# picoexperiment/AutoBub3hs

Hardware: AMD Instinct MI355X
Metric: frames/s end-to-end detect @1280x1024 8-bit (higher is better)
Workload: dtype u8

## Files before the change

autobub3hs_amd/_lib.py:

```python
import ctypes as C
import os
import subprocess

HERE = os.path.dirname(os.path.abspath(__file__))
SO = os.path.join(HERE, "libabub_hip.so")
HEADER = os.path.join(os.path.dirname(HERE), "include", "abub_hip.h")


class Job(C.Structure):
    _fields_ = [("cur", C.c_uint32), ("ref", C.c_uint32), ("model", C.c_uint32), ("out", C.c_uint32)]


def build(force=False):
    srcs = [os.path.join(HERE, "csrc", f) for f in os.listdir(os.path.join(HERE, "csrc"))
            if f.endswith((".hip", ".h", ".hpp")) or f == "Makefile"] + [HEADER]
    stale = force or not os.path.exists(SO) or any(os.path.getmtime(s) > os.path.getmtime(SO) for s in srcs)
    if stale:
        subprocess.check_call(["make", "-C", os.path.join(HERE, "csrc"), "-s"])
    return SO


_vp, _i, _sz = C.c_void_p, C.c_int, C.c_size_t
SIGNATURES = {
    "abub_last_error": (C.c_char_p, []),
    "abub_device_count": (_i, []),
    "abub_device_info": (_i, [_i, C.c_char_p, _i, C.POINTER(_i), C.POINTER(C.c_uint64)]),
    "abub_sigma6_dev": (_i, [_vp, _vp, _sz, _vp]),
    "abub_fill_stack_jobs_dev": (_i, [_vp, _i, _i, _i, _i, _i, _i, _vp]),
    "abub_diff_hist_dev": (_i, [_vp, _vp, _vp, _i, _i, _i, _vp, _vp, _i, _vp]),
    "abub_diff_roi_dev": (_i, [_vp, _vp, _vp, _i, _i, _i, _i, _i, _i, _vp, _vp, _vp]),
    "abub_train_dev": (_i, [_vp, _vp, _i, _i, _i, _vp, _vp, _vp]),
    "abub_pair_hist_dev": (_i, [_vp, _vp, _i, _i, _i, _vp, _vp]),
    "abub_posttrig_dev": (_i, [_vp, _vp, _vp, _vp, _i, _i, _i, _vp, _vp, _vp]),
    "abub_fg_compact_dev": (_i, [_vp, _i, _i, _i, _vp, _vp, _i, _vp, _vp]),
    "abub_fast_path": (_i, [_i]),
    "abub_scratch_release": (_i, [_vp]),
    "abub_bound_counts_dev": (_i, [_vp, C.POINTER(C.c_uint32)]),
    "abub_diff_hist_chained_dev": (_i, [_vp, _vp, _vp, _i, _i, _i, _vp, _i, _i, _vp]),
    "abub_diff_hist_chained_store_dev": (_i, [_vp, _vp, _vp, _i, _i, _i, _vp, _vp, _i, _i, _vp]),
    "abub_k2_set_option": (_i, [C.c_char_p, _i]),
    "abub_k2_deferred_ok": (_i, [_i, _i]),
    "abub_k3_set_option": (_i, [C.c_char_p, _i]),
    "abub_k2_pieces_cap": (_sz, [_i, _i, _i]),
    "abub_png_raw_stride": (_sz, [_i, _i]),
    "abub_png_decode_dev": (_i, [_vp, _sz, _vp, _i, _vp, _i, _vp, _i, _i, _i, _vp, _sz, _vp, _sz, _vp, _sz, _vp, _vp]),
    "abub_diff_hist_chained_deferred_dev": (_i, [_vp, _vp, _vp, _i, _i, _i, _vp, _i, _i, _vp, C.c_uint32, _vp, _vp, _vp]),
    "abub_diff_hist_pieces_dev": (_i, [_vp, _vp, _vp, _i, _i, _i, _vp, _vp, _vp, _vp, _vp]),
    "abub_diff_hist_compact_dev": (_i, [_vp, _vp, _vp, _i, _i, _i, _vp, _vp, _vp, _vp, C.c_uint32, _vp, C.c_uint32, _vp]),
    "abub_posttrig_compact_dev": (_i, [_vp, _vp, _vp, _vp, _i, _i, _i, _vp, _vp, _vp, _vp, C.c_uint32, _vp, C.c_uint32, _vp]),
    "abub_pairs_group_dev": (_i, [_vp, _vp, C.c_uint32, _i, _vp, _vp, _vp, _vp, _vp]),
    "abub_pairs_group_hist_dev": (_i, [_vp, _vp, C.c_uint32, _i, _vp, _vp, _vp, _vp, _vp, _vp, _vp]),
    "abub_fg_compact_pairs_dev": (_i, [_vp, _i, _i, _i, _vp, _vp, C.c_uint32, _vp, _vp]),
    "abub_match_ccorr_dev": (_i, [_vp, _i, _i, _vp, _i, _i, _vp, _vp, _vp]),
    "abub_subsat_hist_dev": (_i, [_vp, _vp, _i, _i, _vp, _vp]),
    "abub_match_ccorr_batch_dev": (_i, [_vp, _i, _i, _vp, _i, _vp, _i, _i, _vp, _vp, _vp]),
    "abub_match_best_batch_dev": (_i, [_vp, _i, _i, _vp, _i, _vp, _i, _i, _vp, _vp, _sz, _vp]),
    "abub_match_best_scratch_bytes": (_sz, [_i, _i, _i, _i, _i]),
    "abub_binarize_thr_dev": (_i, [_vp, _vp, _i, _i, _i, _vp, _vp]),
    "abub_label_blobs_dev": (_i, [_vp, _vp, _vp, C.c_uint32, _i, _i, _i, _vp, _vp, _vp, _vp, C.c_uint32, _vp, _vp, _vp, _vp,
                                  C.c_uint32, _vp, _vp, _sz, _vp]),
    "abub_label_blobs_scratch_bytes": (_sz, [_i, _i, _i, C.c_uint32, _i]),
    "abub_ctx_create": (_i, [C.POINTER(_vp), _i, _i, _i, _i]),
    "abub_ctx_destroy": (None, [_vp]),
    "abub_ctx_train": (_i, [_vp, C.POINTER(_vp), _i, _vp, _vp]),
    "abub_ctx_pair_hist": (_i, [_vp, _vp, _vp, _vp]),
    "abub_ctx_set_model": (_i, [_vp, _vp, _vp]),
    "abub_ctx_upload_stack": (_i, [_vp, C.POINTER(_vp), _i]),
    "abub_ctx_diff_hist_batch": (_i, [_vp, _i, _i, _i, _vp]),
    "abub_ctx_diff_frame": (_i, [_vp, _i, _i, _vp, _vp]),
    "abub_ctx_diff_frame_roi": (_i, [_vp, _i, _i, _i, _i, _i, _i, _vp, _vp]),
    "abub_ctx_posttrig": (_i, [_vp, _i, _vp, _vp]),
    "abub_ctx_foreground": (_i, [_vp, _i, _vp, _i, C.POINTER(_i)]),
    "abub_ctx_match_template": (_i, [_vp, _i, _vp, _i, _i, _vp, _vp]),
    "abub_ctx_subtract_image": (_i, [_vp, _vp, _vp]),
    "abub_ctx_set_image": (_i, [_vp, _vp]),
    "abub_ctx_fetch_image": (_i, [_vp, _vp]),
}

_lib = None


def lib():
    global _lib
    if _lib is None:
        if not os.path.exists(SO):
            raise RuntimeError(
                f"{SO} is missing: build it with `python -c 'import __graft_entry__ as g; g.build()'` "
                "(there is no CPU fallback for the hot path)")
        try:
            import torch
        except ImportError:
            pass
        L = C.CDLL(SO)
        for name, (res, args) in SIGNATURES.items():
            fn = getattr(L, name)
            fn.restype = res
            fn.argtypes = args
        _lib = L
    return _lib


class AbubError(RuntimeError):
    pass


def check(rc, what=""):
    if rc != 0:
        raise AbubError(f"{what} failed rc={rc}: {lib().abub_last_error().decode(errors='replace')}")
```

autobub3hs_amd/csrc/abub_dev.hpp:

```cpp
#pragma once
#include <hip/hip_runtime.h>
#include <stdint.h>
#include <stdio.h>
#include <stdlib.h>
#include <string.h>

#include <map>
#include <mutex>
#include <utility>

#include "../../include/abub_hip.h"

int abub_set_err_(int code, const char *what, hipError_t e);
static int set_err(int code, const char *what, hipError_t e = hipSuccess) { return abub_set_err_(code, what, e); }
#define HIPCHK(x)                                   \
    do {                                            \
        hipError_t e_ = (x);                        \
        if (e_ != hipSuccess)                       \
            return set_err(ABUB_E_HIP, #x, e_);     \
    } while (0)

typedef unsigned short u16x2 __attribute__((ext_vector_type(2)));
typedef short s16x2 __attribute__((ext_vector_type(2)));

// ... 292 lines not shown
                                                     const uint2 *__restrict__ glist, const uint32_t *__restrict__ gcount,
                                                     uint32_t gcap, const int32_t *__restrict__ cthr, uint32_t *pairs,
                                                     uint32_t pcap, uint32_t *pcount, uint32_t slot_base)
{
    __shared__ uint32_t wtot[4], bbase;
    __shared__ uint32_t lh[4][256];
    uint32_t n = *gcount;
    if (n > gcap)
        n = gcap;
    const size_t P = (size_t)W * H;
    const uint32_t ngroups = (uint32_t)W / 4;
    const int tid = threadIdx.x, lane = tid & 63, wv = tid >> 6;
    uint32_t KE = (n + gridDim.x * 256u - 1u) / (gridDim.x * 256u);
    KE = KE < 1u ? 1u : (KE > SUSL_UB ? (uint32_t)SUSL_UB : KE);
    const uint32_t PER = 256u * KE;
#pragma unroll
    for (int q = 0; q < 4; q++)
        lh[wv][4 * lane + q] = 0;
    for (uint32_t e0 = blockIdx.x * PER; e0 < n; e0 += gridDim.x * PER) {
        uint32_t Ov[SUSL_UB], pix0[SUSL_UB], slot[SUSL_UB];
        int thr[SUSL_UB];
        uint32_t c = 0;
        uint32_t job0 = 0xffffffffu;
        {
            const uint32_t ef = e0 + (uint32_t)(wv * 64) * KE;
            if (ef < n)
                job0 = glist[ef].x;
            job0 = (uint32_t)__builtin_amdgcn_readfirstlane((int)job0);
        }
        uint2 ens[SUSL_UB];
        abub_job jbs[SUSL_UB];
#pragma unroll
        for (int u = 0; u < SUSL_UB; u++) {
            const uint32_t e = e0 + (uint32_t)tid * KE + (uint32_t)u;
            ens[u] = make_uint2(0xffffffffu, 0u);
            if ((uint32_t)u < KE && e < n)
                ens[u] = glist[e];
        }
#pragma unroll
        for (int u = 0; u < SUSL_UB; u++)
            jbs[u] = jobs[ens[u].x != 0xffffffffu ? ens[u].x : 0u];
#pragma unroll
        for (int u = 0; u < SUSL_UB; u++) {
            Ov[u] = 0;
            pix0[u] = 0;
            slot[u] = 0;
            thr[u] = 255;
            const uint2 en = ens[u];
            if (en.x != 0xffffffffu) {
                const abub_job jb = jbs[u];
                const int y = (int)(en.y / ngroups), x0 = (int)(en.y % ngroups) * 4;
                uint32_t packed;
                if (KIND == 2)
                    packed = k2_exact_group(frames + (size_t)jb.cur * P, frames + (size_t)jb.ref * P,
                                            sigma6 + (size_t)jb.model * P, y, x0, W, H);
                else
                    packed = k3_exact_group(frames + (size_t)jb.cur * P, mu + (size_t)jb.model * P,
                                            sigma6 + (size_t)jb.model * P, y, x0, W, H);
                if (COMPACT)
                    thr[u] = compact_thr(cthr, jb.out);
#pragma unroll
                for (int q = 0; q < 4; q++) {
                    const uint32_t v = (packed >> (8 * q)) & 0xffu;
                    if (v) {
                        if (en.x == job0)
                            atomicAdd(&lh[wv][v], 1u);
                        else
                            atomicAdd(&hist[(size_t)jb.out * 256 + v], 1u);
                    }
                    c += COMPACT && (int)v > thr[u];
                }
                if (STORE)
                    *reinterpret_cast<uint32_t *>(img + (size_t)jb.out * P + (size_t)y * W + x0) = packed;
                Ov[u] = packed;
                pix0[u] = (uint32_t)(y * W + x0);
                slot[u] = jb.out + slot_base;
            }
        }
        if (job0 != 0xffffffffu) {
            wave_lds_fence();
            const size_t hb = (size_t)jobs[job0].out * 256;
#pragma unroll
            for (int q = 0; q < 4; q++) {
                const uint32_t cnt = lh[wv][4 * lane + q];
                if (cnt) {
                    atomicAdd(&hist[hb + 4 * lane + q], cnt);
                    lh[wv][4 * lane + q] = 0;
                }
            }
            wave_lds_fence();
        }
        if (COMPACT) {
            uint32_t inc = c;
#pragma unroll
            for (int o = 1; o < 64; o <<= 1) {
                const uint32_t t = __shfl_up(inc, o);
                if (lane >= o)
                    inc += t;
            }
            if (lane == 63)
                wtot[wv] = inc;
            __syncthreads();
            if (tid == 0) {
                const uint32_t tot = wtot[0] + wtot[1] + wtot[2] + wtot[3];
                bbase = tot ? atomicAdd(pcount, tot) : 0u;
            }
            __syncthreads();
            uint32_t pos = bbase + inc - c;
            for (int w = 0; w < wv; w++)
                pos += wtot[w];
#pragma unroll
            for (int u = 0; u < SUSL_UB; u++)
#pragma unroll
                for (int q = 0; q < 4; q++) {
                    const uint32_t v = (Ov[u] >> (8 * q)) & 0xffu;
                    if ((int)v > thr[u]) {
                        if (pos < pcap) {
                            pairs[2 * (size_t)pos] = slot[u] | (v << 24);
                            pairs[2 * (size_t)pos + 1] = pix0[u] + q;
                        }
                        ++pos;
                    }
                }
            __syncthreads();
        }
    }
}

static inline int pick_ndw(int W)
{
    if (W < 4 || (W & 3))
        return 0;
    int nd = W / 4;
    for (int ndw = 1; ndw <= 8; ndw++)
        if (nd % ndw == 0 && nd / ndw <= 64)
            return ndw;
    return 0;
}

void *abub_k2_scratch(hipStream_t st, size_t bytes, std::unique_lock<std::mutex> &hold);
static inline void *k2_scratch(hipStream_t st, size_t bytes, std::unique_lock<std::mutex> &hold) { return abub_k2_scratch(st, bytes, hold); }

struct CompactArgs {
    const int32_t *cthr;
    uint32_t *pairs;
    uint32_t cap;
    uint32_t *count;
    uint32_t slot_base;
    int chain_len = 0, chain_stride = 0;
    uint2 *df_pieces = nullptr;
    uint32_t df_cap = 0;
    uint32_t *df_count = nullptr;
    uint8_t *df_incomplete = nullptr;
};
```

autobub3hs_amd/csrc/abub_k2.hip:

```cpp
#include "abub_dev.hpp"

template <int NDW>
struct K2Acc {
    uint32_t pa0[2 * NDW], pa1[2 * NDW], pa2[2 * NDW];
    uint32_t na0[2 * NDW], na1[2 * NDW], na2[2 * NDW];
};
template <int NDW>
struct K2Row {
    uint32_t hp[2 * NDW], hn[2 * NDW];
};

template <int NDW>
__device__ __forceinline__ void k2_planes(const RowIn<NDW> &in, uint32_t (&Xp)[2 * NDW], uint32_t (&Xn)[2 * NDW])
{
#pragma unroll
    for (int d = 0; d < NDW; d++) {
        uint32_t c0 = widen_lo(in.c[d]), c1 = widen_hi(in.c[d]);
        uint32_t r0 = widen_lo(in.r[d]), r1 = widen_hi(in.r[d]);
        uint32_t s0 = widen_lo(in.s[d]), s1 = widen_hi(in.s[d]);
        Xp[2 * d] = pk_subsat(c0, r0 + s0);
        Xn[2 * d] = pk_subsat(r0, c0 + s0);
        Xp[2 * d + 1] = pk_subsat(c1, r1 + s1);
        Xn[2 * d + 1] = pk_subsat(r1, c1 + s1);
    }
// ... 322 lines not shown
        const int dF = Map::segD0(s), dL = Map::segD0(s) + Map::segK(s) - 1;
        uint32_t l = __builtin_amdgcn_update_dpp(0u, m[dL], DPP_WAVE_SHR1, 0xf, 0xf, false);
        uint32_t r = __builtin_amdgcn_update_dpp(0u, m[dF], DPP_WAVE_SHL1, 0xf, 0xf, false);
        uint32_t edgeL = m[dF], edgeR = m[dL];
        if (s > 0)
            edgeL = __builtin_amdgcn_readlane(m[Map::segD0(s - 1) + Map::segK(s - 1) - 1], lastLane);
        if (s + 1 < NSEG)
            edgeR = __builtin_amdgcn_readlane(m[Map::segD0(s + 1)], 0);
        mLs[s] = lane == 0 ? edgeL : l;
        mRs[s] = lane == lastLane ? edgeR : r;
    }
    constexpr int NG = JOB::NG;
    constexpr int GS = JOB::GS;
    static_assert(GS == 2 || NDW == 1, "the segment tables assume pairs of groups");
    uint32_t B[NG];
    uint32_t worst = 0;
#pragma unroll
    for (int g = 0; g < NG; g++) {
        const int g0 = GS * g, g1 = GS * g + GS - 1 < NDW ? GS * g + GS - 1 : NDW - 1;
        const int sg = Map::segOf(g0);
        uint32_t own = m[g0];
#pragma unroll
        for (int q = g0 + 1; q <= g1; q++)
            own += m[q];
        const bool segStart = g0 == Map::segD0(sg), segEnd = g1 == Map::segD0(sg) + Map::segK(sg) - 1;
        const uint32_t M = (segStart ? mLs[sg] : m[g0 - 1]) + own + (segEnd ? mRs[sg] : m[g1 + 1]);
        if constexpr (JOB::CASCADE) {
            const uint32_t s1 = M + J.P[0][par ^ 1][g];
            const uint32_t s2 = s1 + J.P[1][par ^ 1][g];
            const uint32_t s3 = s2 + J.P[2][par ^ 1][g];
            B[g] = s3 + J.P[3][par ^ 1][g];
            J.P[0][par][g] = M;
            J.P[1][par][g] = s1;
            J.P[2][par][g] = s2;
            J.P[3][par][g] = s3;
        } else {
            B[g] = J.P[0][0][g] + M;
            const uint32_t M4 = M << 2;
            J.P[0][0][g] = J.P[1][0][g] + M4;
            J.P[1][0][g] = JOB::PLAIN ? __umul24(M, 6u) + J.P[2][0][g] : pk_madk<6>(M, J.P[2][0][g]);
            if constexpr (JOB::PLAIN) {
                J.P[2][0][g] = J.Mp[par ^ 1][g] + M4;
                J.Mp[par][g] = M;
            } else {
                J.P[2][0][g] = J.P[3][0][g] + M4;
                J.P[3][0][g] = M;
            }
        }
        worst = JOB::PLAIN ? (B[g] > worst ? B[g] : worst) : (worst | B[g]);
    }
    const bool unsure = act && JOB::over(worst);
    if (!(emit && __builtin_amdgcn_ballot_w64(unsure))) {
        J.hot = 0;
        return;
    }
    unsigned long long bm[NG];
    bool mine[NG];
    uint32_t total = 0;
#pragma unroll
    for (int g = 0; g < NG; g++) {
        mine[g] = act && JOB::over(B[g]);
        bm[g] = __builtin_amdgcn_ballot_w64(mine[g]);
        const int nq = GS * g + GS <= NDW ? GS : NDW - GS * g;
        total += (uint32_t)nq * (uint32_t)__builtin_popcountll(bm[g]);
    }
    if (total > 32u) {
        if (J.hot == 0)
            J.mark = J.npend;
        ++J.hot;
    } else
        J.hot = 0;
    if (J.hot >= 4u) {
        J.handover = y - 3;
        J.npend = J.mark;
        return;
    }
    if (J.npend + total > budget) {
        J.handover = y;
        return;
    }
    uint32_t base = J.npend;
#pragma unroll
    for (int g = 0; g < NG; g++) {
        const unsigned long long b = bm[g];
        if (b) {
            const int nq = GS * g + GS <= NDW ? GS : NDW - GS * g;
            const int sg = Map::segOf(GS * g);
            const uint32_t code0 = (uint32_t)y * ngroups + (uint32_t)(map.gbase[sg] + Map::segK(sg) * lane + (GS * g - Map::segD0(sg)));
            const uint32_t below = __builtin_amdgcn_mbcnt_hi((uint32_t)(b >> 32), __builtin_amdgcn_mbcnt_lo((uint32_t)b, 0u));
            if (mine[g]) {
#pragma unroll
                for (int q = 0; q < nq; q++)
                    pend[base + (uint32_t)nq * below + q] = code0 + q;
            }
            base += (uint32_t)nq * (uint32_t)__builtin_popcountll(b);
        }
    }
    J.npend = base;
}

template <bool COMPACT>
__device__ __forceinline__ void k2b_tail(const uint32_t *pend, uint32_t npend, const abub_job jb, const uint8_t *__restrict__ frames,
                                         const uint8_t *__restrict__ sigma6, int W, int H, uint32_t *__restrict__ hist,
                                         uint8_t *__restrict__ diff, const Compact &cp, int lane)
{
    if (npend == 0)
        return;
    wave_lds_fence();
    const size_t P = (size_t)W * H;
    const uint32_t ngroups = (uint32_t)W / 4;
    const uint8_t *cur = frames + (size_t)jb.cur * P;
    const uint8_t *ref = frames + (size_t)jb.ref * P;
    const uint8_t *sg = sigma6 + (size_t)jb.model * P;
    const uint32_t nloop = COMPACT ? (npend + 63u) & ~63u : npend;
#pragma unroll 1
    for (uint32_t e = lane; e < nloop; e += 64) {
        uint32_t packed = 0, pix0 = 0;
        if (e < npend) {
            const uint32_t code = pend[e];
            const int y = (int)(code / ngroups), x0 = (int)(code % ngroups) * 4;
            packed = k2_exact_group(cur, ref, sg, y, x0, W, H);
#pragma unroll
            for (int k = 0; k < 4; k++) {
                const uint32_t d = (packed >> (8 * k)) & 0xffu;
                if (d)
                    atomicAdd(&hist[(size_t)jb.out * 256 + d], 1u);
            }
            if (diff)
                *reinterpret_cast<uint32_t *>(diff + (size_t)jb.out * P + (size_t)y * W + x0) = packed;
            pix0 = (uint32_t)(y * W + x0);
        }
        if (COMPACT) {
            uint32_t c = 0;
#pragma unroll
            for (int k = 0; k < 4; k++)
                c += (int)((packed >> (8 * k)) & 0xffu) > cp.thr;
            uint32_t pos = compact_reserve(cp, c);
#pragma unroll
            for (int k = 0; k < 4; k++)
                compact_put(cp, pos, (packed >> (8 * k)) & 0xffu, pix0 + k);
        }
    }
}

template <int NDW, bool COMPACT>
__global__ __launch_bounds__(64) void k2_bound_scan(const uint8_t *__restrict__ frames,
                                                    const uint8_t *__restrict__ sigma6,
                                                    const abub_job *__restrict__ jobs, int W, int H,
                                                    int rows_per_chunk, int nchunks, uint32_t budget,
                                                    uint2 *__restrict__ units, uint32_t *__restrict__ nunits,
                                                    uint32_t *__restrict__ hist, uint8_t *__restrict__ diff,
                                                    const int32_t *__restrict__ cthr, uint32_t *pairs, uint32_t pcap,
                                                    uint32_t *pcount, uint32_t slot_base, SusList gl,
                                                    uint8_t *__restrict__ incomplete)
{
    constexpr int NP = 2 * NDW;
    __shared__ uint32_t pend[K2B_PEND];
    const int lane = threadIdx.x;
    const int unit = blockIdx.x;
    const int job = unit / nchunks;
    const int chunk = unit - job * nchunks;
    const abub_job jb = jobs[job];
    const size_t P = (size_t)W * H;
    const uint8_t *cur = frames + (size_t)jb.cur * P;
    const uint8_t *ref = frames + (size_t)jb.ref * P;
    const uint8_t *sg = sigma6 + (size_t)jb.model * P;
    const int nl = W / (4 * NDW);
    const bool active = lane < nl;
    const int xoff = active ? lane * 4 * NDW : 0;
    const int y0 = chunk * rows_per_chunk;
    int y1 = y0 + rows_per_chunk;
    if (y1 > H)
        y1 = H;
    const int T = y1 - y0 + 4;
    const uint32_t ngroups = (uint32_t)W / 4;

    ScanMap<NDW, false> map;
    map.init(W);
    K2BoundJob<NDW> J;
#pragma unroll
    for (int g = 0; g < K2BoundJob<NDW>::NG; g++)
#pragma unroll
        for (int q = 0; q < 4; q++)
            J.P[q][0][g] = J.P[q][K2BoundJob<NDW>::CASCADE ? 1 : 0][g] = 0;
    J.npend = J.hot = 0;
    J.jidx = (uint32_t)job;
    J.handover = -1;

    RowIn<NDW> ring[2];
    k2_load_row<NDW>(ring[0], cur, ref, sg, reflect101(y0 - 2, H), W, xoff);
    const int Tpad = (T + 1) & ~1;
    for (int t = 0; t < Tpad && J.handover < 0; t += 2) {
#pragma unroll
        for (int u = 0; u < 2; u++) {
            const int tt = t + u;
            int tn = tt + 1 < T ? tt + 1 : T - 1;
            k2_load_row<NDW>(ring[u ^ 1], cur, ref, sg, reflect101(y0 - 2 + tn, H), W, xoff);
            if (J.handover < 0) {
                uint32_t Xp[NP], Xn[NP];
                k2_planes<NDW>(ring[u], Xp, Xn);
                uint32_t m[NDW];
#pragma unroll
                for (int g = 0; g < NDW; g++)
                    m[g] = (Xp[2 * g] + Xn[2 * g]) + (Xp[2 * g + 1] + Xn[2 * g + 1]);
                k2b_row<NDW, false>(J, u, m, tt >= 4 && tt < T, y0 + tt - 4, map, lane, ngroups, budget, pend, gl);
            }
        }
    }
    if (J.handover >= 0)
        k2b_hand_over(units, nunits, (uint32_t)unit, J.handover, y1, lane, incomplete, (uint32_t)job);
    if (J.npend) {
        wave_lds_fence();
        uint32_t gb = 0;
        if (sus_reserve(J.npend, gl.list, gl.count, gl.cap, gb, lane)) {
            sus_copy_out(pend, J.npend, J.jidx, gl.list, gb, lane);
            return;
        }
    }
    Compact cp;
    cp.pairs = COMPACT ? pairs : nullptr;
    cp.count = pcount;
    cp.cap = pcap;
    cp.slot = jb.out + slot_base;
    cp.thr = COMPACT ? compact_thr(cthr, jb.out) : 255;
    k2b_tail<COMPACT>(pend, J.npend, jb, frames, sigma6, W, H, hist, diff, cp, lane);
}

#define K2C_MAXW 8
#ifndef K2C_DEFAULT_WG
#define K2C_DEFAULT_WG 1
#endif
#ifndef K2C_DEFAULT_SYNC
#define K2C_DEFAULT_SYNC 0
#endif
template <int NDW, int K, bool SPLIT, int PF = 1>
__global__ __launch_bounds__(64 * K2C_MAXW) void k2_sad_chain(const uint8_t *__restrict__ frames,
                                                   const uint8_t *__restrict__ sigma6,
                                                   const abub_job *__restrict__ jobs, int L, int S, int nwgs, int W,
                                                   int H, int rows_per_chunk, int nchunks, uint32_t budget,
                                                   uint2 *__restrict__ units, uint32_t *__restrict__ nunits,
                                                   uint32_t *__restrict__ hist, uint8_t *__restrict__ diff, SusList gl,
                                                   int syncD, uint8_t *__restrict__ incomplete)
{
    using Job = K2BoundJob<NDW, false, true>;
    extern __shared__ uint32_t k2c_lds[];
    const int NW = (int)(blockDim.x >> 6);
    const int lane = (int)(threadIdx.x & 63u);
    const int wave = __builtin_amdgcn_readfirstlane((int)(threadIdx.x >> 6));
    uint32_t(*pend)[K2B_PEND] = reinterpret_cast<uint32_t(*)[K2B_PEND]>(k2c_lds + (size_t)wave * K * K2B_PEND);
    const int progBase = NW * K * K2B_PEND;
#define K2C_PUBLISH(V)                                                                                         \
    {                                                                                                          \
        if (NW > 1 && lane == 0)                                                                               \
            __hip_atomic_store(&k2c_lds[progBase + wave], (uint32_t)(V), __ATOMIC_RELAXED, __HIP_MEMORY_SCOPE_WORKGROUP); \
    }
    const int chunk = blockIdx.x % nchunks;
    const int bs = blockIdx.x / nchunks;
    const int blk = bs / nwgs;
    int wg = bs - blk * nwgs;
    int r = 0, nr = 0, ns = 0;
    for (r = 0; r < S; r++) {
        nr = (L - r + S - 1) / S;
        ns = (nr + K - 1) / K;
        const int nw = (ns + NW - 1) / NW;
        if (wg < nw)
            break;
        wg -= nw;
    }
    const int slot = wg * NW + wave;
    if (r >= S || slot >= ns) {
        K2C_PUBLISH(0x7fffffff);
        return;
    }
    const int k = nr - slot * K < K ? nr - slot * K : K;
    Job J[K];
    abub_job jb[K];
    const uint32_t jidx0 = (uint32_t)(blk * L + r + S * slot * K);
#pragma unroll
    for (int t = 0; t < K; t++)
        jb[t] = jobs[jidx0 + (uint32_t)(S * (t < k ? t : k - 1))];
    const int y0 = chunk * rows_per_chunk;
    int y1 = y0 + rows_per_chunk;
    if (y1 > H)
        y1 = H;
    bool chained = true;
#pragma unroll
    for (int t = 1; t < K; t++)
        if (t < k && (jb[t].ref != jb[t - 1].cur || jb[t].model != jb[0].model))
            chained = false;
    if (!chained) {
#pragma unroll
        for (int t = 0; t < K; t++)
            if (t < k)
                k2b_hand_over(units, nunits, (jidx0 + (uint32_t)(S * t)) * (uint32_t)nchunks + (uint32_t)chunk, y0, y1, lane, incomplete,
                              jidx0 + (uint32_t)(S * t));
        K2C_PUBLISH(0x7fffffff);
        return;
    }
    const size_t P = (size_t)W * H;
    const uint8_t *fp[K + 1];
    fp[0] = frames + (size_t)jb[0].ref * P;
#pragma unroll
    for (int t = 0; t < K; t++)
        fp[t + 1] = frames + (size_t)jb[t].cur * P;
    const uint8_t *sg = sigma6 + (size_t)jb[0].model * P;
    ScanMap<NDW, SPLIT> map;
    map.init(W);
    const int T = y1 - y0 + 4;
    const uint32_t ngroups = (uint32_t)W / 4;
#pragma unroll
    for (int t = 0; t < K; t++) {
#pragma unroll
        for (int g = 0; g < Job::NG; g++)
#pragma unroll
            for (int q = 0; q < 4; q++)
                J[t].P[q][0][g] = 0;
#pragma unroll
        for (int g = 0; g < Job::NG; g++)
            J[t].Mp[0][g] = J[t].Mp[1][g] = 0;
        J[t].npend = J[t].hot = 0;
        J[t].handover = t < k ? -1 : 0x7fffffff;
    }
    constexpr int RING = PF + 1, U = (RING % 2 == 0) ? RING : 2 * RING;
    uint32_t raw[RING][K + 2][NDW];
#define K2C_LOAD(SL, Y)                                                                       \
    {                                                                                         \
        const size_t o_ = (size_t)(Y) * W;                                                    \
        _Pragma("unroll") for (int f = 0; f <= K; f++) map.load(raw[SL][f], fp[f] + o_, lane); \
        map.load(raw[SL][K + 1], sg + o_, lane);                                              \
    }
#pragma unroll
    for (int q = 0; q < PF; q++) {
        const int tq = q < T ? q : T - 1;
        K2C_LOAD(q, reflect101(y0 - 2 + tq, H));
    }
    const int Tpad = (T + U - 1) / U * U;
    for (int t0 = 0; t0 < Tpad; t0 += U) {
        bool all_done = true;
#pragma unroll
        for (int t = 0; t < K; t++)
            all_done = all_done && J[t].handover >= 0;
        if (all_done)
            break;
        if (NW > 1) {
            K2C_PUBLISH(t0);
            if (syncD > 0) {
                for (;;) {
                    int mn = 0x7fffffff;
                    for (int w = 0; w < NW; w++) {
                        const int pw_ = (int)__hip_atomic_load(&k2c_lds[progBase + w], __ATOMIC_RELAXED, __HIP_MEMORY_SCOPE_WORKGROUP);
                        mn = pw_ < mn ? pw_ : mn;
                    }
                    if (t0 <= __builtin_amdgcn_readfirstlane(mn) + syncD)
                        break;
                    __builtin_amdgcn_s_sleep(8);
                }
            }
        }
#pragma unroll
        for (int uu = 0; uu < U; uu++) {
            const int tt = t0 + uu;
            const int tn = tt + PF < T ? tt + PF : T - 1;
            K2C_LOAD((uu + PF) % RING, reflect101(y0 - 2 + tn, H));
            const int u = uu % RING;
            const int par = uu & 1;
            const bool emit = tt >= 4 && tt < T;
            const int y = y0 + tt - 4;
            uint32_t s8[2 * NDW];
#pragma unroll
            for (int d = 0; d < NDW; d++) {
                s8[2 * d] = widen8_lo(raw[u][K + 1][d]);
                s8[2 * d + 1] = widen8_hi(raw[u][K + 1][d]);
            }
#pragma unroll
            for (int h = 1; h <= K; h += 2) {
                const bool ja = J[h - 1].handover < 0, jc = h < K && J[h < K ? h : K - 1].handover < 0;
                if (!(ja || jc))
                    continue;
                uint32_t HI[NDW], LO[NDW], nS[NDW];
#pragma unroll
                for (int d = 0; d < NDW; d++) {
                    const uint32_t r0 = widen8_lo(raw[u][h][d]), r1 = widen8_hi(raw[u][h][d]);
                    HI[d] = pack8(pk_addsat(r0, s8[2 * d]), pk_addsat(r1, s8[2 * d + 1]));
                    LO[d] = pack8(pk_subsat(r0, s8[2 * d]), pk_subsat(r1, s8[2 * d + 1]));
                    nS[d] = 0u - __builtin_amdgcn_sad_u8(HI[d], LO[d], 0u);
                }
#pragma unroll
                for (int q = 0; q < 2; q++) {
                    const int t = h - 1 + q, fc = q ? h + 1 : h - 1;
                    if (t >= K)
                        continue;
                    if (J[t].handover < 0) {
                        uint32_t m[NDW];
#pragma unroll
                        for (int d = 0; d < NDW; d++)
                            m[d] = __builtin_amdgcn_sad_u8(raw[u][fc][d], LO[d], __builtin_amdgcn_sad_u8(raw[u][fc][d], HI[d], nS[d]));
                        k2b_row<NDW, SPLIT>(J[t], par, m, emit, y, map, lane, ngroups, budget, pend[t], gl);
                    }
                }
            }
        }
    }
#undef K2C_LOAD
    K2C_PUBLISH(0x7fffffff);
#undef K2C_PUBLISH
    uint32_t tot = 0;
#pragma unroll
    for (int t = 0; t < K; t++) {
        if (t < k) {
            if (J[t].handover >= 0)
                k2b_hand_over(units, nunits, (jidx0 + (uint32_t)(S * t)) * (uint32_t)nchunks + (uint32_t)chunk, J[t].handover, y1, lane,
                              incomplete, jidx0 + (uint32_t)(S * t));
            tot += J[t].npend;
        }
    }
    if (tot == 0)
        return;
    wave_lds_fence();
    uint32_t gb = 0;
    if (sus_reserve(tot, gl.list, gl.count, gl.cap, gb, lane)) {
#pragma unroll
        for (int t = 0; t < K; t++)
            if (t < k) {
                sus_copy_out(pend[t], J[t].npend, jidx0 + (uint32_t)(S * t), gl.list, gb, lane);
                gb += J[t].npend;
            }
        return;
    }
    Compact cp;
    cp.pairs = nullptr;
    cp.count = nullptr;
    cp.cap = 0;
    cp.slot = 0;
    cp.thr = 255;
#pragma unroll
    for (int t = 0; t < K; t++)
        if (t < k)
// ... 69 lines not shown
{
    dim3 grid((unsigned)njobs * nchunks), block(64);
#define K2_LAUNCH(ST, CO)                                                                                        \
    hipLaunchKernelGGL((k2_rows<NDW, ST, PF, CO>), grid, block, 0, st, frames, sigma6, jobs, W, H, R, nchunks, \
                       hist, diff, ca.cthr, ca.pairs, ca.cap, ca.count, ca.slot_base, nullptr, nullptr)
    if (ca.cthr) {
        if (diff)
            K2_LAUNCH(true, true);
        else
            K2_LAUNCH(false, true);
    } else {
        if (diff)
            K2_LAUNCH(true, false);
        else
            K2_LAUNCH(false, false);
    }
#undef K2_LAUNCH
}

struct K2Options {
    int bound = 1;
    int chain = -1;
    int budget = 512;
    int pf = 1;
    int scanpf = -1;
    int split = 1;
    int list = 0;
    int wg = -1;
    int sync = -1;
    int chunks = 0;
    bool loaded = false;
};
static K2Options g_k2opt;
static std::mutex g_k2optMu;
static K2Options k2_options()
{
    std::lock_guard<std::mutex> lock(g_k2optMu);
    if (!g_k2opt.loaded) {
        if (const char *e = getenv("ABUB_K2_BOUND"))
            g_k2opt.bound = atoi(e);
        if (const char *e = getenv("ABUB_K2_CHAIN"))
            g_k2opt.chain = atoi(e);
        if (const char *e = getenv("ABUB_K2_BUDGET"))
            if (atoi(e) > 0)
                g_k2opt.budget = atoi(e);
        if (const char *e = getenv("ABUB_K2_PF"))
            g_k2opt.pf = atoi(e);
        if (const char *e = getenv("ABUB_K2_SPLIT"))
            g_k2opt.split = atoi(e);
        if (const char *e = getenv("ABUB_K2_LIST"))
            g_k2opt.list = atoi(e);
        if (const char *e = getenv("ABUB_K2_WG"))
            g_k2opt.wg = atoi(e);
        if (const char *e = getenv("ABUB_K2_SYNC"))
            g_k2opt.sync = atoi(e);
        if (const char *e = getenv("ABUB_K2_SCANPF"))
            g_k2opt.scanpf = atoi(e);
        if (const char *e = getenv("ABUB_K2_CHUNKS"))
            if (atoi(e) >= 0 && atoi(e) <= K_MAX_CHUNKS)
                g_k2opt.chunks = atoi(e);
        g_k2opt.loaded = true;
    }
    return g_k2opt;
}

extern "C" int abub_k2_set_option(const char *name, int value)
{
    if (!name)
        return set_err(ABUB_E_INVALID, "abub_k2_set_option: null name");
    (void)k2_options();
    std::lock_guard<std::mutex> lock(g_k2optMu);
    if (!strcmp(name, "bound"))
        g_k2opt.bound = value;
    else if (!strcmp(name, "chain"))
        g_k2opt.chain = value;
    else if (!strcmp(name, "budget") && value > 0)
        g_k2opt.budget = value;
    else if (!strcmp(name, "pf"))
        g_k2opt.pf = value;
    else if (!strcmp(name, "split"))
        g_k2opt.split = value;
    else if (!strcmp(name, "list"))
        g_k2opt.list = value;
    else if (!strcmp(name, "wg"))
        g_k2opt.wg = value;
    else if (!strcmp(name, "sync"))
        g_k2opt.sync = value;
    else if (!strcmp(name, "scanpf"))
        g_k2opt.scanpf = value;
    else if (!strcmp(name, "chunks") && value >= 0 && value <= K_MAX_CHUNKS)
        g_k2opt.chunks = value;
    else
        return set_err(ABUB_E_INVALID, "abub_k2_set_option: unknown option or bad value");
    return ABUB_OK;
}

template <int NDW>
static int launch_k2_rows(const uint8_t *frames, const uint8_t *sigma6, const abub_job *jobs,
                           int njobs, int W, int H, int R, int nchunks, uint32_t *hist, uint8_t *diff,
                           const CompactArgs &ca, hipStream_t st)
{
    const K2Options opt = k2_options();
    if (opt.bound && (size_t)H * (size_t)(W / 4) < ((size_t)1 << 32) && H < 65536) {
        if (diff)
            HIPCHK(hipMemsetAsync(diff, 0, (size_t)njobs * (size_t)W * (size_t)H, st));
        const size_t nunits = (size_t)njobs * nchunks;
        const uint32_t budget = (uint32_t)(opt.budget < K2B_PEND ? opt.budget : K2B_PEND);
        const size_t unitCap = nunits * (size_t)((R + K2B_SUB - 1) / K2B_SUB);
        const size_t unitBytes = (unitCap * sizeof(uint2) + 255) & ~(size_t)255;
        size_t gcap = (size_t)njobs * 1024;
        gcap = gcap < ((size_t)1 << 16) ? ((size_t)1 << 16) : (gcap > ((size_t)1 << 24) ? ((size_t)1 << 24) : gcap);
        if (!opt.list)
            gcap = 0;
        const size_t bytes = 256 + unitBytes + gcap * sizeof(uint2) + 256;
        std::unique_lock<std::mutex> hold;
        uint8_t *scr = (uint8_t *)k2_scratch(st, bytes, hold);
        if (!scr)
            return set_err(ABUB_E_HIP, "abub_diff_hist_dev: scratch allocation failed");
        uint32_t *counters = (uint32_t *)scr;
        uint2 *units = (uint2 *)(scr + 256);
        uint32_t *npieces = counters;
        const bool deferred = ca.df_pieces != nullptr;
        if (deferred) {
            if (diff || ca.cthr || !ca.df_count || !ca.df_incomplete || (size_t)ca.df_cap < unitCap)
                return set_err(ABUB_E_INVALID, "deferred pieces: trigger-only launches with a list of abub_k2_pieces_cap() entries");
            units = ca.df_pieces;
            npieces = ca.df_count;
            HIPCHK(hipMemsetAsync(npieces, 0, sizeof(uint32_t), st));
            HIPCHK(hipMemsetAsync(ca.df_incomplete, 0, (size_t)njobs, st));
        }
        SusList gl;
        gl.list = gcap ? (uint2 *)(scr + 256 + unitBytes) : nullptr;
        gl.count = counters + 32;
        gl.cap = (uint32_t)gcap;
        const unsigned tgrid = (unsigned)((gcap + 256 * SUSL_UB - 1) / (256 * SUSL_UB) < 2048 ? (gcap + 256 * SUSL_UB - 1) / (256 * SUSL_UB) : 2048);
        HIPCHK(hipMemsetAsync(counters, 0, 256, st));
        const int L = ca.chain_len, S = ca.chain_stride;
        const int chainK = opt.chain < 0 ? 4 : opt.chain;
        if (chainK >= 2 && L > 0 && S > 0 && S <= 8 && njobs % L == 0 && !ca.cthr) {
            const int Kc = chainK >= 3 ? 4 : 2;
            const int NW = opt.wg < 0 ? K2C_DEFAULT_WG : (opt.wg < 1 ? 1 : (opt.wg > K2C_MAXW ? K2C_MAXW : opt.wg));
            int nwgs = 0;
            for (int r = 0; r < S; r++) {
                const int nr = (L - r + S - 1) / S;
                const int ns = nr > 0 ? (nr + Kc - 1) / Kc : 0;
                nwgs += (ns + NW - 1) / NW;
            }
            const dim3 grid((unsigned)((size_t)(njobs / L) * nwgs * nchunks));
            const size_t ldsBytes = ((size_t)NW * Kc * K2B_PEND + 64) * sizeof(uint32_t);
            const int syncD = opt.sync < 0 ? K2C_DEFAULT_SYNC : opt.sync;
            constexpr bool CAN_SPLIT = NDW >= 5 && NDW <= 7;
            const bool split = CAN_SPLIT && opt.split;
            const bool pf2 = NDW == 5 && split && Kc == 4 && (opt.scanpf < 0 || opt.scanpf == 2);
#define K2C_ARGS frames, sigma6, jobs, L, S, nwgs, W, H, R, nchunks, budget, units, npieces, hist, diff, gl, syncD, ca.df_incomplete
#define K2C_LAUNCH_SP(KK, SP, PFD) \
    hipLaunchKernelGGL((k2_sad_chain<NDW, KK, SP, PFD>), grid, dim3(64 * NW), ldsBytes, st, K2C_ARGS)
#define K2C_LAUNCH(KK)                                                                                              \
    if (split) {                                                                                                    \
        K2C_LAUNCH_SP(KK, CAN_SPLIT, 1);                                                                            \
    } else {                                                                                                        \
        K2C_LAUNCH_SP(KK, false, 1);                                                                                \
    }
            if (pf2) {
                if constexpr (NDW == 5)
                    K2C_LAUNCH_SP(4, true, 2);
            } else if (Kc == 4) {
                K2C_LAUNCH(4);
            } else {
                K2C_LAUNCH(2);
            }
#undef K2C_LAUNCH_SP
#undef K2C_ARGS
#undef K2C_LAUNCH
        } else {
#define K2S_LAUNCH(CO)                                                                                              \
    hipLaunchKernelGGL((k2_bound_scan<NDW, CO>), dim3((unsigned)nunits), dim3(64), 0, st, frames, sigma6, jobs, W, H, \
                       R, nchunks, budget, units, npieces, hist, diff, ca.cthr, ca.pairs, ca.cap, ca.count,         \
                       ca.slot_base, gl, ca.df_incomplete)
            if (ca.cthr) {
                K2S_LAUNCH(true);
            } else {
                K2S_LAUNCH(false);
            }
#undef K2S_LAUNCH
        }
        if (gl.list) {
#define K2T_LAUNCH(CO, ST)                                                                                          \
    hipLaunchKernelGGL((sus_tail_list<2, CO, ST>), dim3(tgrid), dim3(256), 0, st, frames, (const uint8_t *)nullptr,  \
                       sigma6, jobs, W, H, hist, diff, gl.list, gl.count, gl.cap, ca.cthr, ca.pairs, ca.cap, ca.count, \
                       ca.slot_base)
            if (ca.cthr) {
                if (diff) {
                    K2T_LAUNCH(true, true);
                } else {
                    K2T_LAUNCH(true, false);
                }
            } else {
                if (diff) {
                    K2T_LAUNCH(false, true);
                } else {
                    K2T_LAUNCH(false, false);
                }
            }
#undef K2T_LAUNCH
        }
        if (deferred)
            return ABUB_OK;
        const unsigned g3 = (unsigned)(unitCap < 4096 ? unitCap : 4096);
#define K2R_LAUNCH(ST, CO)                                                                                          \
    hipLaunchKernelGGL((k2_rows<NDW, ST, 1, CO>), dim3(g3), dim3(64), 0, st, frames, sigma6, jobs, W, H, R, nchunks, \
                       hist, diff, ca.cthr, ca.pairs, ca.cap, ca.count, ca.slot_base, units, counters)
        if (ca.cthr) {
            if (diff)
                K2R_LAUNCH(true, true);
            else
                K2R_LAUNCH(false, true);
        } else {
            if (diff)
                K2R_LAUNCH(true, false);
            else
                K2R_LAUNCH(false, false);
        }
#undef K2R_LAUNCH
        return ABUB_OK;
    }
    if (ca.df_pieces)
        return set_err(ABUB_E_INVALID, "deferred pieces need the bound-and-verify pass (option \"bound\" on)");
    if (opt.pf == 2)
        launch_k2_rows_pf<NDW, 2>(frames, sigma6, jobs, njobs, W, H, R, nchunks, hist, diff, ca, st);
    else
        launch_k2_rows_pf<NDW, 1>(frames, sigma6, jobs, njobs, W, H, R, nchunks, hist, diff, ca, st);
    return ABUB_OK;
}

static int k2_auto_rows(int njobs, int H)
{
    int nch = 8;
    if ((long long)njobs * nch < 8192)
        nch = (8192 + njobs - 1) / njobs;
    const int chunks = k2_options().chunks;
    if (chunks > 0)
        nch = chunks;
    nch = (nch + 7) / 8 * 8;
    int R = (H + nch - 1) / nch;
    if (R < 16)
        R = 16;
    return R;
}

static int diff_hist_impl(const uint8_t *frames, const uint8_t *sigma6, const abub_job *jobs, int njobs,
                          int W, int H, uint32_t *hist, uint8_t *diff, int rows_per_chunk,
                          const CompactArgs &ca, void *stream)
{
    if (!frames || !sigma6 || !jobs || !hist || W <= 0 || H <= 0 || njobs < 0 || rows_per_chunk < 0)
        return set_err(ABUB_E_INVALID, "abub_diff_hist_dev: bad arguments");
    if (njobs == 0)
        return ABUB_OK;
    hipStream_t st = (hipStream_t)stream;
    HIPCHK(hipMemsetAsync(hist, 0, (size_t)njobs * 256 * sizeof(uint32_t), st));
    int ndw = pick_ndw(W);
    if (ndw) {
        const int R = rows_per_chunk ? rows_per_chunk : k2_auto_rows(njobs, H);
        int nchunks = (H + R - 1) / R;
        int rc = ABUB_OK;
        switch (ndw) {
        case 1: rc = launch_k2_rows<1>(frames, sigma6, jobs, njobs, W, H, R, nchunks, hist, diff, ca, st); break;
        case 2: rc = launch_k2_rows<2>(frames, sigma6, jobs, njobs, W, H, R, nchunks, hist, diff, ca, st); break;
        case 3: rc = launch_k2_rows<3>(frames, sigma6, jobs, njobs, W, H, R, nchunks, hist, diff, ca, st); break;
        case 4: rc = launch_k2_rows<4>(frames, sigma6, jobs, njobs, W, H, R, nchunks, hist, diff, ca, st); break;
        case 5: rc = launch_k2_rows<5>(frames, sigma6, jobs, njobs, W, H, R, nchunks, hist, diff, ca, st); break;
        case 6: rc = launch_k2_rows<6>(frames, sigma6, jobs, njobs, W, H, R, nchunks, hist, diff, ca, st); break;
        case 7: rc = launch_k2_rows<7>(frames, sigma6, jobs, njobs, W, H, R, nchunks, hist, diff, ca, st); break;
        default: rc = launch_k2_rows<8>(frames, sigma6, jobs, njobs, W, H, R, nchunks, hist, diff, ca, st); break;
        }
        if (rc != ABUB_OK)
            return rc;
    } else {
        if (ca.cthr)
            return set_err(ABUB_E_INVALID, "fused compaction needs the fast path (W % 4 == 0, W <= 2048)");
        abub_job dummy = {0, 0, 0, 0};
        dim3 grid((W + G_TW - 1) / G_TW, (H + G_TH - 1) / G_TH, njobs), block(256);
        if (grid.z > 65535)
            return set_err(ABUB_E_INVALID, "abub_diff_hist_dev: too many jobs for the generic kernel");
        hipLaunchKernelGGL(k2_generic, grid, block, 0, st, frames, sigma6, jobs, dummy, 0, W, H, 0, 0,
                           W, H, hist, diff);
    }
    HIPCHK(hipGetLastError());
    hipLaunchKernelGGL(k_hist_bin0, dim3(njobs), dim3(64), 0, st, hist, (uint32_t)((size_t)W * H));
    HIPCHK(hipGetLastError());
    return ABUB_OK;
}

extern "C" int abub_diff_hist_dev(const uint8_t *frames, const uint8_t *sigma6, const abub_job *jobs,
                                  int njobs, int W, int H, uint32_t *hist, uint8_t *diff,
                                  int rows_per_chunk, void *stream)
{
    CompactArgs ca = {nullptr, nullptr, 0, nullptr, 0};
    return diff_hist_impl(frames, sigma6, jobs, njobs, W, H, hist, diff, rows_per_chunk, ca, stream);
}

extern "C" int abub_diff_hist_chained_dev(const uint8_t *frames, const uint8_t *sigma6, const abub_job *jobs,
                                          int njobs, int W, int H, uint32_t *hist, int chain_len, int chain_stride,
                                          void *stream)
{
    if (chain_len < 0 || chain_stride < 0)
        return set_err(ABUB_E_INVALID, "abub_diff_hist_chained_dev: bad arguments");
    CompactArgs ca = {nullptr, nullptr, 0, nullptr, 0};
    ca.chain_len = chain_len;
    ca.chain_stride = chain_stride;
    return diff_hist_impl(frames, sigma6, jobs, njobs, W, H, hist, nullptr, 0, ca, stream);
}

extern "C" int abub_diff_hist_chained_store_dev(const uint8_t *frames, const uint8_t *sigma6, const abub_job *jobs,
                                                int njobs, int W, int H, uint32_t *hist, uint8_t *diff, int chain_len,
                                                int chain_stride, void *stream)
{
    if (chain_len < 0 || chain_stride < 0 || !diff)
        return set_err(ABUB_E_INVALID, "abub_diff_hist_chained_store_dev: bad arguments");
    CompactArgs ca = {nullptr, nullptr, 0, nullptr, 0};
    ca.chain_len = chain_len;
    ca.chain_stride = chain_stride;
    return diff_hist_impl(frames, sigma6, jobs, njobs, W, H, hist, diff, 0, ca, stream);
}

extern "C" size_t abub_k2_pieces_cap(int njobs, int W, int H)
{
    if (njobs <= 0 || H <= 0)
        return 0;
    const int R = k2_auto_rows(njobs, H), nchunks = (H + R - 1) / R;
    return (size_t)njobs * nchunks * (size_t)((R + K2B_SUB - 1) / K2B_SUB);
}

extern "C" int abub_k2_deferred_ok(int W, int H)
{
    return W > 0 && H > 0 && H < 65536 && (size_t)H * (size_t)(W / 4) < ((size_t)1 << 32) && pick_ndw(W) != 0 &&
           k2_options().bound != 0;
}

extern "C" int abub_diff_hist_chained_deferred_dev(const uint8_t *frames, const uint8_t *sigma6, const abub_job *jobs, int njobs,
                                                   int W, int H, uint32_t *hist, int chain_len, int chain_stride,
                                                   void *pieces, uint32_t pieces_cap, uint32_t *npieces,
                                                   uint8_t *incomplete, void *stream)
{
    if (chain_len < 0 || chain_stride < 0 || !pieces || !npieces || !incomplete || !pick_ndw(W) || !k2_options().bound)
        return set_err(ABUB_E_INVALID, "abub_diff_hist_chained_deferred_dev: bad arguments (or no bound-and-verify pass for this width)");
    CompactArgs ca = {nullptr, nullptr, 0, nullptr, 0};
    ca.chain_len = chain_len;
    ca.chain_stride = chain_stride;
    ca.df_pieces = (uint2 *)pieces;
    ca.df_cap = pieces_cap;
    ca.df_count = npieces;
    ca.df_incomplete = incomplete;
    return diff_hist_impl(frames, sigma6, jobs, njobs, W, H, hist, nullptr, 0, ca, stream);
}

template <int NDW>
static void launch_pieces(const uint8_t *frames, const uint8_t *sigma6, const abub_job *jobs, int W, int H, int R, int nchunks,
                          uint32_t *hist, const uint2 *pieces, const uint32_t *npieces, const uint8_t *want, unsigned grid,
                          hipStream_t st)
{
    hipLaunchKernelGGL((k2_rows<NDW, false, 1, false>), dim3(grid), dim3(64), 0, st, frames, sigma6, jobs, W, H, R, nchunks, hist,
                       (uint8_t *)nullptr, (const int32_t *)nullptr, (uint32_t *)nullptr, 0u, (uint32_t *)nullptr, 0u, pieces,
                       npieces, want);
}

extern "C" int abub_diff_hist_pieces_dev(const uint8_t *frames, const uint8_t *sigma6, const abub_job *jobs, int njobs, int W,
                                         int H, uint32_t *hist, const void *pieces_, const uint32_t *npieces,
                                         const uint8_t *want, void *stream)
{
    const uint2 *pieces = (const uint2 *)pieces_;
    if (!frames || !sigma6 || !jobs || !hist || !pieces || !npieces || !want || njobs <= 0 || W <= 0 || H <= 0)
        return set_err(ABUB_E_INVALID, "abub_diff_hist_pieces_dev: bad arguments");
    const int ndw = pick_ndw(W);
    if (!ndw)
        return set_err(ABUB_E_INVALID, "abub_diff_hist_pieces_dev: no fast path for this width");
    hipStream_t st = (hipStream_t)stream;
    const int R = k2_auto_rows(njobs, H), nchunks = (H + R - 1) / R;
    const size_t cap = abub_k2_pieces_cap(njobs, W, H);
    const unsigned grid = (unsigned)(cap < 4096 ? cap : 4096);
    switch (ndw) {
    case 1: launch_pieces<1>(frames, sigma6, jobs, W, H, R, nchunks, hist, pieces, npieces, want, grid, st); break;
    case 2: launch_pieces<2>(frames, sigma6, jobs, W, H, R, nchunks, hist, pieces, npieces, want, grid, st); break;
    case 3: launch_pieces<3>(frames, sigma6, jobs, W, H, R, nchunks, hist, pieces, npieces, want, grid, st); break;
    case 4: launch_pieces<4>(frames, sigma6, jobs, W, H, R, nchunks, hist, pieces, npieces, want, grid, st); break;
    case 5: launch_pieces<5>(frames, sigma6, jobs, W, H, R, nchunks, hist, pieces, npieces, want, grid, st); break;
    case 6: launch_pieces<6>(frames, sigma6, jobs, W, H, R, nchunks, hist, pieces, npieces, want, grid, st); break;
    case 7: launch_pieces<7>(frames, sigma6, jobs, W, H, R, nchunks, hist, pieces, npieces, want, grid, st); break;
    default: launch_pieces<8>(frames, sigma6, jobs, W, H, R, nchunks, hist, pieces, npieces, want, grid, st); break;
    }
    HIPCHK(hipGetLastError());
    hipLaunchKernelGGL(k_hist_bin0, dim3(njobs), dim3(64), 0, st, hist, (uint32_t)((size_t)W * H), want);
    HIPCHK(hipGetLastError());
    return ABUB_OK;
}

extern "C" int abub_fast_path(int W) { return pick_ndw(W) != 0; }

extern "C" int abub_diff_hist_compact_dev(const uint8_t *frames, const uint8_t *sigma6, const abub_job *jobs,
                                          int njobs, int W, int H, uint32_t *hist, uint8_t *diff,
                                          const int32_t *cthr, uint32_t *pairs, uint32_t cap,
                                          uint32_t *count, uint32_t slot_base, void *stream)
{
    if (!cthr || !pairs || !count || cap == 0)
        return set_err(ABUB_E_INVALID, "abub_diff_hist_compact_dev: bad arguments");
    CompactArgs ca = {cthr, pairs, cap, count, slot_base};
    return diff_hist_impl(frames, sigma6, jobs, njobs, W, H, hist, diff, 0, ca, stream);
}

extern "C" int abub_diff_roi_dev(const uint8_t *cur, const uint8_t *ref, const uint8_t *sigma6, int W,
                                 int H, int rx, int ry, int rw, int rh, uint8_t *diff, uint32_t *hist,
                                 void *stream)
{
    if (!cur || !ref || !sigma6 || !diff || !hist || W <= 0 || H <= 0 || rx < 0 || ry < 0 ||
        rw < 0 || rh < 0 || rx + rw > W || ry + rh > H)
        return set_err(ABUB_E_INVALID, "abub_diff_roi_dev: bad arguments");
    hipStream_t st = (hipStream_t)stream;
    size_t P = (size_t)W * H;
    HIPCHK(hipMemsetAsync(diff, 0, P, st));
    HIPCHK(hipMemsetAsync(hist, 0, 256 * sizeof(uint32_t), st));
    if (rw > 0 && rh > 0) {
        abub_job jb = {0, 0, 0, 0};
        dim3 grid((rw + G_TW - 1) / G_TW, (rh + G_TH - 1) / G_TH, 1), block(256);
        ptrdiff_t dref = ref - cur;
        if (dref % (ptrdiff_t)P != 0 || dref < 0)
            return set_err(ABUB_E_INVALID, "abub_diff_roi_dev: ref must follow cur in the same slab at a multiple of W*H");
        jb.ref = (uint32_t)(dref / (ptrdiff_t)P);
        hipLaunchKernelGGL(k2_generic, grid, block, 0, st, cur, sigma6, (const abub_job *)nullptr, jb, 1,
                           W, H, rx, ry, rw, rh, hist, diff);
        HIPCHK(hipGetLastError());
    }
    hipLaunchKernelGGL(k_hist_bin0, dim3(1), dim3(64), 0, st, hist, (uint32_t)P);
    HIPCHK(hipGetLastError());
    return ABUB_OK;
}
```

autobub3hs_amd/csrc/abub_misc.hip:

```cpp
#include "abub_dev.hpp"

static thread_local char g_err[256] = "";

extern "C" const char *abub_last_error(void) { return g_err; }

int abub_set_err_(int code, const char *what, hipError_t e)
{
    if (e != hipSuccess)
        snprintf(g_err, sizeof g_err, "%s: %s", what, hipGetErrorString(e));
    else
        snprintf(g_err, sizeof g_err, "%s", what);
    return code;
}

extern "C" int abub_device_count(void)
{
    int n = 0;
    if (hipGetDeviceCount(&n) != hipSuccess)
        return 0;
    return n;
}

extern "C" int abub_device_info(int device, char *name, int name_cap, int *cus, uint64_t *hbm_bytes)
{
    hipDeviceProp_t p;
    HIPCHK(hipGetDeviceProperties(&p, device));
    if (name && name_cap > 0)
        snprintf(name, name_cap, "%s (%s)", p.name, p.gcnArchName);
    if (cus)
        *cus = p.multiProcessorCount;
    if (hbm_bytes)
        *hbm_bytes = p.totalGlobalMem;
    return ABUB_OK;
}

__global__ void k_sigma6(const uint8_t *__restrict__ s, uint8_t *__restrict__ o, size_t n)
{
    size_t i = (size_t)blockIdx.x * blockDim.x + threadIdx.x;
    size_t stride = (size_t)gridDim.x * blockDim.x;
    for (; i < n; i += stride) {
        int v = 6 * (int)s[i];
        o[i] = (uint8_t)(v > 255 ? 255 : v);
    }
}

extern "C" int abub_sigma6_dev(const uint8_t *sigma, uint8_t *sigma6, size_t n, void *stream)
{
    if (!sigma || !sigma6)
        return set_err(ABUB_E_INVALID, "abub_sigma6_dev: null pointer");
    if (n == 0)
        return ABUB_OK;
    int blocks = (int)((n + 255) / 256);
    if (blocks > 4096)
        blocks = 4096;
    hipLaunchKernelGGL(k_sigma6, dim3(blocks), dim3(256), 0, (hipStream_t)stream, sigma, sigma6, n);
    HIPCHK(hipGetLastError());
    return ABUB_OK;
}

__global__ void k_fill_stack_jobs(abub_job *jobs, int nstacks, int F, int first, int count, int off,
                                  int nmodels)
{
    int j = blockIdx.x * blockDim.x + threadIdx.x;
    if (j >= nstacks * count)
        return;
    int s = j / count, n = j % count;
    int i = first + n;
    int r = i - off;
    if (r < 0)
        r = 0;
    abub_job jb;
    jb.cur = (uint32_t)(s * F + i);
    jb.ref = (uint32_t)(s * F + r);
    jb.model = (uint32_t)(s % nmodels);
    jb.out = (uint32_t)j;
    jobs[j] = jb;
}

extern "C" int abub_fill_stack_jobs_dev(abub_job *jobs, int nstacks, int F, int first, int count,
                                        int ref_offset, int nmodels, void *stream)
{
    if (!jobs || nstacks < 0 || F <= 0 || first < 0 || count < 0 || first + count > F ||
        ref_offset < 0 || nmodels <= 0)
        return set_err(ABUB_E_INVALID, "abub_fill_stack_jobs_dev: bad arguments");
    int n = nstacks * count;
    if (n == 0)
        return ABUB_OK;
    hipLaunchKernelGGL(k_fill_stack_jobs, dim3((n + 255) / 256), dim3(256), 0, (hipStream_t)stream,
                       jobs, nstacks, F, first, count, ref_offset, nmodels);
    HIPCHK(hipGetLastError());
    return ABUB_OK;
}

struct K2ScratchBuf {
    void *p = nullptr;
    size_t n = 0;
};
static std::mutex g_scratchMu;
static std::map<std::pair<int, hipStream_t>, K2ScratchBuf> g_scratch;

void *abub_k2_scratch(hipStream_t st, size_t bytes, std::unique_lock<std::mutex> &hold)
{
    int dev = 0;
    if (hipGetDevice(&dev) != hipSuccess)
        return nullptr;
    hold = std::unique_lock<std::mutex>(g_scratchMu);
    K2ScratchBuf &b = g_scratch[std::make_pair(dev, st)];
    if (b.n < bytes) {
        if (b.p) {
            (void)hipStreamSynchronize(st);
            (void)hipFree(b.p);
            b.p = nullptr;
            b.n = 0;
        }
        const size_t want = bytes + bytes / 4;
        if (hipMalloc(&b.p, want) != hipSuccess) {
            b.p = nullptr;
            return nullptr;
        }
        b.n = want;
    }
    return b.p;
}

extern "C" int abub_bound_counts_dev(void *stream, uint32_t counts[2])
{
    if (!counts)
        return set_err(ABUB_E_INVALID, "abub_bound_counts_dev: null pointer");
    counts[0] = counts[1] = 0;
    int dev = 0;
    HIPCHK(hipGetDevice(&dev));
    hipStream_t st = (hipStream_t)stream;
    std::lock_guard<std::mutex> lock(g_scratchMu);
    auto it = g_scratch.find(std::make_pair(dev, st));
    if (it == g_scratch.end() || !it->second.p)
        return ABUB_OK;
    uint32_t c[64];
    HIPCHK(hipStreamSynchronize(st));
    HIPCHK(hipMemcpy(c, it->second.p, sizeof c, hipMemcpyDeviceToHost));
    counts[0] = c[0];
    counts[1] = c[32];
    return ABUB_OK;
}

extern "C" int abub_scratch_release(void *stream)
{
    int dev = 0;
    HIPCHK(hipGetDevice(&dev));
    hipStream_t st = (hipStream_t)stream;
    std::lock_guard<std::mutex> lock(g_scratchMu);
    auto it = g_scratch.find(std::make_pair(dev, st));
    if (it == g_scratch.end())
        return ABUB_OK;
    (void)hipStreamSynchronize(st);
    if (it->second.p)
        (void)hipFree(it->second.p);
    g_scratch.erase(it);
    return ABUB_OK;
}

__global__ __launch_bounds__(256) void k1_welford(const uint8_t *__restrict__ frames,
                                                  const uint32_t *__restrict__ idx, int N, size_t P,
                                                  uint8_t *__restrict__ mu, uint8_t *__restrict__ sigma)
{
    size_t px = (size_t)blockIdx.x * blockDim.x + threadIdx.x;
    if (px >= P)
        return;
    float mean = 0.f, m2 = 0.f;
    for (int k = 0; k < N; k++) {
        size_t f = idx ? idx[k] : (uint32_t)k;
        float x = (float)frames[f * P + px];
        float delta = x - mean;
        mean = mean + delta / (float)(k + 1);
        m2 = m2 + delta * (x - mean);
    }
    float var = m2 / (float)(N - 1);
    float sd = sqrtf(var);
    int isd = (sd != sd) ? 0 : (int)sd;
    sigma[px] = (uint8_t)isd;
    mu[px] = (uint8_t)(int)mean;
}

__global__ __launch_bounds__(256) void k1_welford4(const uint8_t *__restrict__ frames,
                                                   const uint32_t *__restrict__ idx, int N, size_t P,
                                                   uint8_t *__restrict__ mu,
                                                   uint8_t *__restrict__ sigma)
{
    size_t q = (size_t)blockIdx.x * blockDim.x + threadIdx.x;
    if (q * 4 >= P)
        return;
    float mean[4] = {0.f, 0.f, 0.f, 0.f}, m2[4] = {0.f, 0.f, 0.f, 0.f};
    for (int k = 0; k < N; k++) {
        size_t f = idx ? idx[k] : (uint32_t)k;
        uint32_t w = reinterpret_cast<const uint32_t *>(frames + f * P)[q];
        float kk = (float)(k + 1);
#pragma unroll
        for (int b = 0; b < 4; b++) {
            float x = (float)((w >> (8 * b)) & 0xffu);
            float delta = x - mean[b];
            mean[b] = mean[b] + delta / kk;
            m2[b] = m2[b] + delta * (x - mean[b]);
        }
    }
    uint32_t om = 0, os = 0;
    float nm1 = (float)(N - 1);
#pragma unroll
    for (int b = 0; b < 4; b++) {
        float sd = sqrtf(m2[b] / nm1);
        int isd = (sd != sd) ? 0 : (int)sd;
        os |= (uint32_t)(isd & 0xff) << (8 * b);
        om |= (uint32_t)((int)mean[b] & 0xff) << (8 * b);
    }
    reinterpret_cast<uint32_t *>(mu)[q] = om;
    reinterpret_cast<uint32_t *>(sigma)[q] = os;
}

extern "C" int abub_train_dev(const uint8_t *frames, const uint32_t *idx, int N, int W, int H,
                              uint8_t *mu, uint8_t *sigma, void *stream)
{
    if (!frames || !mu || !sigma || N <= 0 || W <= 0 || H <= 0)
        return set_err(ABUB_E_INVALID, "abub_train_dev: bad arguments");
    size_t P = (size_t)W * H;
    hipStream_t st = (hipStream_t)stream;
    if ((P & 3) == 0) {
        size_t nq = P / 4;
        hipLaunchKernelGGL(k1_welford4, dim3((unsigned)((nq + 255) / 256)), dim3(256), 0, st, frames,
                           idx, N, P, mu, sigma);
    } else {
        hipLaunchKernelGGL(k1_welford, dim3((unsigned)((P + 255) / 256)), dim3(256), 0, st, frames, idx,
                           N, P, mu, sigma);
    }
    HIPCHK(hipGetLastError());
    return ABUB_OK;
}

__global__ __launch_bounds__(256) void k1b_pair_hist(const uint8_t *__restrict__ frames,
                                                     const abub_job *__restrict__ pairs, size_t P,
                                                     uint32_t *__restrict__ hist)
{
    __shared__ uint32_t lh[256];
    const abub_job jb = pairs[blockIdx.y];
    const uint8_t *f1 = frames + (size_t)jb.cur * P;
// ... 405 lines not shown
```

autobub3hs_amd/hip.py:

```python
import torch

from . import _lib


def _ptr(t):
    return None if t is None else t.data_ptr()


def _stream():
    return torch.cuda.current_stream().cuda_stream


def _need_cuda(*ts):
    for t in ts:
        if t is not None and not t.is_cuda:
            raise _lib.AbubError("device-pointer launcher called with a CPU tensor (no CPU fallback)")
        if t is not None and not t.is_contiguous():
            raise _lib.AbubError("tensor must be contiguous")


def sigma6(sigma):
    _need_cuda(sigma)
    out = torch.empty_like(sigma)
    _lib.check(_lib.lib().abub_sigma6_dev(_ptr(sigma), _ptr(out), sigma.numel(), _stream()), "abub_sigma6_dev")
    return out


def stack_jobs(nstacks, F, first, count, ref_offset, nmodels, device):
    jobs = torch.empty((nstacks * count, 4), dtype=torch.int32, device=device)
    _lib.check(_lib.lib().abub_fill_stack_jobs_dev(_ptr(jobs), nstacks, F, first, count, ref_offset,
                                                   nmodels, _stream()), "abub_fill_stack_jobs_dev")
    return jobs


def make_jobs(rows, device):
    return torch.tensor(list(rows), dtype=torch.int64).to(torch.int32).reshape(-1, 4).to(device)


def diff_hist(frames, sigma6_, jobs, W, H, store=False, rows_per_chunk=0, hist=None, diff=None, chain=None):
    _need_cuda(frames, sigma6_, jobs)
    n = jobs.shape[0]
    if hist is None:
        hist = torch.empty((n, 256), dtype=torch.int32, device=frames.device)
    if store and diff is None:
        diff = torch.empty((n, H, W), dtype=torch.uint8, device=frames.device)
    if chain is not None:
        assert rows_per_chunk == 0
        if store:
            _lib.check(_lib.lib().abub_diff_hist_chained_store_dev(_ptr(frames), _ptr(sigma6_), _ptr(jobs), n, W, H,
                                                                   _ptr(hist), _ptr(diff), int(chain[0]), int(chain[1]),
                                                                   _stream()), "abub_diff_hist_chained_store_dev")
            return hist, diff
        _lib.check(_lib.lib().abub_diff_hist_chained_dev(_ptr(frames), _ptr(sigma6_), _ptr(jobs), n, W, H, _ptr(hist),
                                                         int(chain[0]), int(chain[1]), _stream()),
                   "abub_diff_hist_chained_dev")
        return hist, None
    _lib.check(_lib.lib().abub_diff_hist_dev(_ptr(frames), _ptr(sigma6_), _ptr(jobs), n, W, H, _ptr(hist),
                                             _ptr(diff) if store else None, rows_per_chunk, _stream()),
               "abub_diff_hist_dev")
    return hist, (diff if store else None)


def diff_hist_deferred(frames, sigma6_, jobs, W, H, chain):
    _need_cuda(frames, sigma6_, jobs)
    n = jobs.shape[0]
    hist = torch.empty((n, 256), dtype=torch.int32, device=frames.device)
    cap = int(_lib.lib().abub_k2_pieces_cap(n, W, H))
    pieces = torch.empty((max(cap, 1), 2), dtype=torch.int32, device=frames.device)
    npieces = torch.zeros((1,), dtype=torch.int32, device=frames.device)
    incomplete = torch.empty((n,), dtype=torch.uint8, device=frames.device)
    _lib.check(_lib.lib().abub_diff_hist_chained_deferred_dev(_ptr(frames), _ptr(sigma6_), _ptr(jobs), n, W, H, _ptr(hist),
                                                              int(chain[0]), int(chain[1]), _ptr(pieces), cap, _ptr(npieces),
                                                              _ptr(incomplete), _stream()),
               "abub_diff_hist_chained_deferred_dev")
    return hist, (pieces, npieces, incomplete)


def diff_hist_pieces(frames, sigma6_, jobs, W, H, hist, state, want):
    _need_cuda(frames, sigma6_, jobs, want)
    pieces, npieces, _ = state
    _lib.check(_lib.lib().abub_diff_hist_pieces_dev(_ptr(frames), _ptr(sigma6_), _ptr(jobs), jobs.shape[0], W, H, _ptr(hist),
                                                    _ptr(pieces), _ptr(npieces), _ptr(want), _stream()),
               "abub_diff_hist_pieces_dev")
    return hist


def k2_set_option(name, value):
    _lib.check(_lib.lib().abub_k2_set_option(name.encode(), int(value)), "abub_k2_set_option")


def k3_set_option(name, value):
    _lib.check(_lib.lib().abub_k3_set_option(name.encode(), int(value)), "abub_k3_set_option")


def bound_counts(stream=None):
    import ctypes as C

    st = torch.cuda.current_stream().cuda_stream if stream is None else stream
    out = (C.c_uint32 * 2)()
    _lib.check(_lib.lib().abub_bound_counts_dev(st, out), "abub_bound_counts_dev")
    return int(out[0]), int(out[1])


def diff_roi(slab, cur, ref, sigma6_, W, H, roi):
    _need_cuda(slab, sigma6_)
    rx, ry, rw, rh = roi
    diff = torch.empty((H, W), dtype=torch.uint8, device=slab.device)
    hist = torch.empty((256,), dtype=torch.int32, device=slab.device)
    P = W * H
    base = slab.data_ptr()
    _lib.check(_lib.lib().abub_diff_roi_dev(base + cur * P, base + ref * P, _ptr(sigma6_), W, H, rx, ry, rw, rh,
                                            _ptr(diff), _ptr(hist), _stream()), "abub_diff_roi_dev")
    return diff, hist


def train(frames, W, H, idx=None):
    _need_cuda(frames, idx)
    N = frames.shape[0] if idx is None else idx.numel()
    mu = torch.empty((H, W), dtype=torch.uint8, device=frames.device)
    sg = torch.empty((H, W), dtype=torch.uint8, device=frames.device)
    _lib.check(_lib.lib().abub_train_dev(_ptr(frames), _ptr(idx), N, W, H, _ptr(mu), _ptr(sg), _stream()),
               "abub_train_dev")
    return mu, sg


def pair_hist(frames, pairs, W, H):
    _need_cuda(frames, pairs)
    n = pairs.shape[0]
    hist = torch.empty((n, 256), dtype=torch.int32, device=frames.device)
    _lib.check(_lib.lib().abub_pair_hist_dev(_ptr(frames), _ptr(pairs), n, W, H, _ptr(hist), _stream()),
               "abub_pair_hist_dev")
    return hist


def posttrig(frames, mu, sigma6_, jobs, W, H, store=True):
    _need_cuda(frames, mu, sigma6_, jobs)
    n = jobs.shape[0]
    hist = torch.empty((n, 256), dtype=torch.int32, device=frames.device)
    img = torch.empty((n, H, W), dtype=torch.uint8, device=frames.device) if store else None
    _lib.check(_lib.lib().abub_posttrig_dev(_ptr(frames), _ptr(mu), _ptr(sigma6_), _ptr(jobs), n, W, H,
                                            _ptr(hist), _ptr(img), _stream()), "abub_posttrig_dev")
    return hist, img


def fg_compact(img, thr, cap):
    _need_cuda(img, thr)
    n, H, W = img.shape
    idx = torch.empty((n, cap), dtype=torch.int32, device=img.device)
    cnt = torch.empty((n,), dtype=torch.int32, device=img.device)
    _lib.check(_lib.lib().abub_fg_compact_dev(_ptr(img), n, W, H, _ptr(thr), _ptr(idx), cap, _ptr(cnt),
                                              _stream()), "abub_fg_compact_dev")
    return idx, cnt



def binarize_thr(hist, tozero, W, H):
    _need_cuda(hist, tozero)
    n = tozero.numel()
    thr = torch.empty((n,), dtype=torch.int32, device=hist.device)
    _lib.check(_lib.lib().abub_binarize_thr_dev(_ptr(hist), _ptr(tozero), n, W, H, _ptr(thr), _stream()),
               "abub_binarize_thr_dev")
    return thr


def label_blobs(offsets, idx, val, thr, min_box_area, W, H, cap=None, comp=True, in_cap=None):
    _need_cuda(offsets, idx, val, thr, min_box_area)
    n = thr.numel()
    dev = idx.device
    in_cap = int(idx.numel()) if in_cap is None else int(in_cap)
    cap = max(in_cap, 1) if cap is None else int(cap)
    L = _lib.lib()
    need = int(L.abub_label_blobs_scratch_bytes(n, W, H, in_cap, 1 if comp else 0))
    scratch = torch.empty((max(need, 1),), dtype=torch.uint8, device=dev)
    out = {"kept_off": torch.empty((n + 1,), dtype=torch.int32, device=dev),
           "kept_idx": torch.empty((cap,), dtype=torch.int32, device=dev),
           "ncomp": torch.empty((n,), dtype=torch.int32, device=dev),
           "nkept_comp": torch.empty((n,), dtype=torch.int32, device=dev),
           "comp_off": torch.empty((n + 1,), dtype=torch.int32, device=dev),
           "comp": torch.empty((cap, 6), dtype=torch.int32, device=dev) if comp else None,
           "stats": torch.empty((4,), dtype=torch.int32, device=dev)}
    _lib.check(L.abub_label_blobs_dev(_ptr(offsets), _ptr(idx), _ptr(val), in_cap, n, W, H, _ptr(thr), _ptr(min_box_area),
                                      _ptr(out["kept_off"]), _ptr(out["kept_idx"]), cap, _ptr(out["ncomp"]),
                                      _ptr(out["nkept_comp"]), _ptr(out["comp_off"]), _ptr(out["comp"]), cap if comp else 0,
                                      _ptr(out["stats"]), _ptr(scratch), scratch.numel(), _stream()),
               "abub_label_blobs_dev")
    return out

def png_parse(data, W, H):
    import struct
    if len(data) < 33 or data[:8] != b"\x89PNG\r\n\x1a\n":
        return None
    o, segs, pal, hdr, end = 8, [], None, None, False
    while not end and o + 12 <= len(data):
        ln, = struct.unpack(">I", data[o:o + 4])
        typ = data[o + 4:o + 8]
        if o + 12 + ln > len(data):
            return None
        if typ == b"IHDR" and ln >= 13:
            hdr = struct.unpack(">IIBBBBB", data[o + 8:o + 21])
        elif typ == b"PLTE":
            pal = data[o + 8:o + 8 + ln]
        elif typ == b"IDAT":
            segs.append((o + 8, ln))
        elif typ == b"IEND":
            end = True
        o += 12 + ln
    if hdr is None or not segs or hdr[0] != W or hdr[1] != H or hdr[2] != 8 or hdr[3] not in (0, 3) or hdr[6] != 0:
        return None
    lut = None
    if hdr[3] == 3:
        n = min(len(pal or b"") // 3, 256)
        lut = bytes(((pal[3 * i] * 9797 + pal[3 * i + 1] * 19234 + pal[3 * i + 2] * 3737 + 16384) >> 15) & 255 if i < n else 0
                    for i in range(256))
    return segs, lut


def png_decode(files, W, H, device="cuda:0"):
    import numpy as np
    n = len(files)
    frames_np = np.zeros((max(n, 1), 8), dtype=np.uint32)
    segs, luts, blob, zoff = [], [], bytearray(), 0
    status_pre = np.zeros(n, dtype=np.int32)
    P = W * H
    for i, data in enumerate(files):
        parsed = png_parse(data, W, H)
        base = len(blob)
        if parsed is None:
            status_pre[i] = -1
# ... 59 lines not shown
```

autobub3hs_amd/host.py:

```python
import ctypes as C
import os
import subprocess

import numpy as np

HERE = os.path.dirname(os.path.abspath(__file__))
SO = os.path.join(HERE, "libabub_host.so")

_u8p = C.POINTER(C.c_uint8)
_u32p = C.POINTER(C.c_uint32)
_u64p = C.POINTER(C.c_uint64)
_ip = C.POINTER(C.c_int)
_fp = C.POINTER(C.c_float)
_dp = C.POINTER(C.c_double)
_vp, _i, _s = C.c_void_p, C.c_int, C.c_char_p
SIGNATURES = {
    "abh_run_new": (_vp, []),
    "abh_run_open": (_vp, [_i, _s, _s, _s]),
    "abh_run_free": (None, [_vp]),
    "abh_run_events": (_s, [_vp]),
    "abh_run_frames": (_s, [_vp, _s, _i]),
    "abh_run_image": (_i, [_vp, _s, _s, _u8p, _i, _ip, _ip]),
    "abh_run_add_event": (_i, [_vp, _s, _i, _u8p, _i, _i, _i, _u8p]),
    "abh_train": (_i, [_vp, _i, _ip, _ip, _u8p, _u8p]),
    "abh_train_device": (_i, [_vp, _i, _ip, _ip, _u8p, _u8p, _i, _dp]),
    "abh_set_model": (_i, [_vp, _i, _u8p, _u8p, _i, _i, _i]),
    "abh_probe_frame_stats": (_i, [_vp, _s, _i, _u8p, _i, _i, _i, _dp]),
    "abh_run_batched": (_i, [_vp, _i, _s, _s, _s] + [_i] * 7 + [_dp]),
    "abh_analyze": (_i, [_vp, _s, _i, _s]),
    "abh_last_error": (_s, [_vp]),
    "abh_run_last": (_vp, [_vp]),
    "abh_result_state": (None, [_vp, _ip]),
    "abh_result_error": (_s, [_vp]),
    "abh_result_ndesc": (_i, [_vp, _i]),
    "abh_result_desc": (None, [_vp, _i, _i, _dp]),
    "abh_result_ndz": (_i, [_vp, _i]),
    "abh_result_dz": (C.c_float, [_vp, _i, _i]),
    "abh_result_dzdt": (C.c_float, [_vp, _i]),
    "abh_result_drdt": (C.c_float, [_vp, _i]),
    "abh_imdecode": (_i, [_u8p, _i, _u8p, _i, _ip, _ip]),
    "abh_png_walk": (_i, [_u8p, _i, _i, _i, _u32p, _i, _ip, _ip, _u8p]),
    "abh_imwrite": (_i, [_s, _u8p, _i, _i]),
    "abh_write_header": (None, [_s, _s, _i, _i]),
    "abh_event_to_file": (_i, [_vp, _s, _i, _i, _s, _s, _s, _i]),
    "abh_writer_probe": (None, [_s, _s, _i, _i, _i, _ip, _ip, _ip, _ip, _dp]),
    "abh_contours": (_i, [_u32p, _i, _i, _i, _ip, _ip, _i, _i]),
    "abh_binarize_threshold": (_i, [_u32p, _i, _i]),
    "abh_entropy": (C.c_float, [_u32p, _i, _i]),
    "abh_blob_stats": (None, [_ip, _i, _dp]),
    "abh_best_match": (None, [_u64p, _u64p, _i, _i, _u8p, _i, _i, _fp, _fp]),
    "abh_sig_new": (_vp, []),
    "abh_sig_free": (None, [_vp]),
    "abh_sig_eval": (C.c_double, [_vp, _u32p, _i, _i, _i, _ip]),
    "abh_pipe_new": (_vp, [_i] * 6 + [_ip, _i, _s]),
    "abh_pipe_free": (None, [_vp]),
    "abh_pipe_error": (_s, []),
    "abh_pipe_set_sigma": (None, [_vp, _vp]),
    "abh_pipe_run": (_i, [_vp] * 5),
    "abh_pipe_run_host": (_i, [_vp] * 4),
    "abh_pipe_stack": (_vp, [_vp, _i]),
    "abh_pipe_timing": (_i, [_vp, _dp]),
    "abh_pipe_set_option": (_i, [_vp, _s, _i]),
    "abh_pipe_blob_stats": (None, [_vp, _dp]),
    "abh_pipe_bellows": (None, [_vp, _dp]),
}
_lib = None


def build(force=False):
    from . import _lib as hiplib

    hiplib.build(force)
    subprocess.check_call(["make", "-C", os.path.join(HERE, "host"), "-s"])
    return SO


def lib():
    global _lib
    if _lib is None:
        if not os.path.exists(SO):
            raise RuntimeError(f"{SO} is missing: run __graft_entry__.build()")
        from . import _lib as hiplib

        hiplib.lib()
        L = C.CDLL(SO)
        for name, (res, args) in SIGNATURES.items():
            fn = getattr(L, name)
            fn.restype = res
            fn.argtypes = args
        _lib = L
    return _lib


DESC_KEYS = ("x", "y", "w", "h", "area", "radius", "m00", "m10", "m01", "cx", "cy")


def _read_result(res, with_dz):
    L = lib()
    o = (C.c_int * 6)()
    L.abh_result_state(res, o)
    state = {"trig": o[1], "status": o[2], "ok": bool(o[4]), "loc_thres": o[3]}
    bubbles = []
    buf = (C.c_double * len(DESC_KEYS))()
    for b in range(o[5]):
        descs = []
        for d in range(L.abh_result_ndesc(res, b)):
            L.abh_result_desc(res, b, d, buf)
            dd = dict(zip(DESC_KEYS, list(buf)))
            for k in ("x", "y", "w", "h"):
                dd[k] = int(dd[k])
            descs.append(dd)
        bub = {"desc": descs, "dzdt": L.abh_result_dzdt(res, b), "drdt": L.abh_result_drdt(res, b)}
        if with_dz:
            bub["dz"] = [L.abh_result_dz(res, b, i) for i in range(L.abh_result_ndz(res, b))]
        bubbles.append(bub)
    return o[0], state, bubbles, L.abh_result_error(res).decode()


class Run:

    def __init__(self, kind=None, run_folder="", image_folder="Images", image_format="cam%d_image%u.png"):
        L = lib()
        if kind is None:
            self._h = L.abh_run_new()
        else:
            self._h = L.abh_run_open(0 if kind == "raw" else 1, run_folder.encode(), image_folder.encode(),
                                     image_format.encode())
            if not self._h:
                raise RuntimeError(f"cannot open run source {run_folder!r} (status -10 upstream)")

    def events(self):
        return [e for e in lib().abh_run_events(self._h).decode().split("\n") if e]

    def frames(self, event, cam):
        return [f for f in lib().abh_run_frames(self._h, str(event).encode(), cam).decode().split("\n") if f]

    def image(self, event, frame, cap=1 << 22):
        buf = np.empty(cap, np.uint8)
        w, h = C.c_int(), C.c_int()
        rc = lib().abh_run_image(self._h, str(event).encode(), frame.encode(), buf.ctypes.data_as(_u8p), cap,
                                 C.byref(w), C.byref(h))
        img = buf[: w.value * h.value].reshape(h.value, w.value).copy() if w.value * h.value else None
        return rc, img

    def close(self):
        if self._h:
            lib().abh_run_free(self._h)
            self._h = None

    def __del__(self):
        try:
            self.close()
        except Exception:
            pass

    def add_event(self, event, cam, frames, ok=None):
        frames = np.ascontiguousarray(frames, dtype=np.uint8)
        F, H, W = frames.shape
        okp = None
        if ok is not None:
            ok = np.ascontiguousarray(ok, dtype=np.uint8)
            okp = ok.ctypes.data_as(_u8p)
        lib().abh_run_add_event(self._h, str(event).encode(), cam, frames.ctypes.data_as(_u8p), F, W, H, okp)
        self._shape = (H, W)

    def train(self, cam, shape=None):
        H, W = shape if shape is not None else self._shape
        mu = np.zeros((H, W), np.uint8)
        sg = np.zeros((H, W), np.uint8)
        st, tss = C.c_int(), C.c_int()
        rc = lib().abh_train(self._h, cam, C.byref(st), C.byref(tss), mu.ctypes.data_as(_u8p), sg.ctypes.data_as(_u8p))
        if rc != 0:
            raise RuntimeError(lib().abh_last_error(self._h).decode())
        return st.value, tss.value, mu, sg

    def train_on_gpu(self, ncams, shape=None):
        H, W = shape if shape is not None else self._shape
        L = lib()
        mu = np.zeros((ncams, H, W), np.uint8)
        sg = np.zeros((ncams, H, W), np.uint8)
        st = np.zeros(ncams, np.int32)
        tss = np.zeros(ncams, np.int32)
        stats = np.zeros(4, np.float64)
        rc = L.abh_train_device(self._h, ncams, st.ctypes.data_as(_ip), tss.ctypes.data_as(_ip), mu.ctypes.data_as(_u8p),
                                sg.ctypes.data_as(_u8p), H * W, stats.ctypes.data_as(_dp))
        if rc < 0:
            raise RuntimeError(L.abh_last_error(self._h).decode())
        self.train_path = "device" if rc == 0 else "host"
        self.train_stats = {"frames_gpu_decoded": int(stats[0]), "frames_host_decoded": int(stats[1]),
                            "decode_launches": int(stats[2]), "seconds": float(stats[3])}
        return [(int(st[c]), int(tss[c]), mu[c], sg[c]) for c in range(ncams)]

    def set_model(self, cam, mu, sigma, tss):
        mu = np.ascontiguousarray(mu, dtype=np.uint8)
        sigma = np.ascontiguousarray(sigma, dtype=np.uint8)
        H, W = mu.shape
        lib().abh_set_model(self._h, cam, mu.ctypes.data_as(_u8p), sigma.ctypes.data_as(_u8p), W, H, int(tss))

    def probe_frame_stats(self, event, cam, imgs):
        L = lib()
        imgs = np.ascontiguousarray(imgs, dtype=np.uint8)
        n, H, W = imgs.shape
        out = np.zeros((n, 3), np.float64)
        rc = L.abh_probe_frame_stats(self._h, str(event).encode(), cam, imgs.ctypes.data_as(_u8p), n, W, H,
                                     out.ctypes.data_as(_dp))
        if rc != 0:
            raise RuntimeError(f"abh_probe_frame_stats rc={rc}: " + L.abh_last_error(self._h).decode())
        return out

    def run_batched(self, ncams, outdir, run_number, frame_offset, maskdir="", ngpus=1, nthreads=16, decode_threads=16,
                    batch_mb=0, shard=(0, 1)):
        L = lib()
        st = (C.c_double * 13)()
        rc = L.abh_run_batched(self._h, ncams, maskdir.encode(), outdir.encode(), run_number.encode(), frame_offset, ngpus,
                               nthreads, decode_threads, batch_mb, shard[0], shard[1], st)
        if rc != 0:
# ... 15 lines not shown
    src = np.frombuffer(data, np.uint8)
    out = np.empty(cap, np.uint8)
    w, h = C.c_int(), C.c_int()
    rc = L.abh_imdecode(src.ctypes.data_as(_u8p), len(src), out.ctypes.data_as(_u8p), cap, C.byref(w), C.byref(h))
    if rc != 0:
        return None
    return out[: w.value * h.value].reshape(h.value, w.value).copy()


def png_walk(data, W, H, cap=4096):
    L = lib()
    src = np.frombuffer(data, np.uint8)
    segs = (C.c_uint32 * (2 * cap))()
    n, pal = C.c_int(), C.c_int()
    lut = np.zeros(256, np.uint8)
    if not L.abh_png_walk(src.ctypes.data_as(_u8p), len(src), W, H, segs, cap, C.byref(n), C.byref(pal), lut.ctypes.data_as(_u8p)):
        return None
    return [(segs[2 * i], segs[2 * i + 1]) for i in range(min(n.value, cap))], (lut.tobytes() if pal.value else None)


def imwrite(path, img):
    L = lib()
    img = np.ascontiguousarray(img, dtype=np.uint8)
    return L.abh_imwrite(path.encode(), img.ctypes.data_as(_u8p), img.shape[1], img.shape[0]) == 0


def write_header(outdir, run_number, frame_offset, ncams):
    lib().abh_write_header(outdir.encode(), run_number.encode(), frame_offset, ncams)


def event_to_file(run, event, actual_event_number, ncams, outdir, run_number, frame_offset, maskdir=""):
    rc = lib().abh_event_to_file(run._h, str(event).encode(), int(actual_event_number), ncams, maskdir.encode(),
                                 outdir.encode(), run_number.encode(), frame_offset)
    if rc != 0:
        raise RuntimeError("abh_event_to_file failed")


def writer_probe(outdir, run_number, frame_offset, event, cams):
    L = lib()
    n = len(cams)
    status = (C.c_int * n)(*[c[0] for c in cams])
    frame0 = (C.c_int * n)(*[c[1] for c in cams])
    nbub = (C.c_int * n)(*[len(c[2]) for c in cams])
    nd = [len(b) for c in cams for b in c[2]]
    ndesc = (C.c_int * max(1, len(nd)))(*nd)
    rows = [float(v) for c in cams for b in c[2] for d in b for v in d]
    desc = (C.c_double * max(1, len(rows)))(*rows)
    L.abh_writer_probe(outdir.encode(), run_number.encode(), frame_offset, n, event, status, frame0, nbub, ndesc, desc)


def contours_from_indices(idx, W, H):
    idx = np.ascontiguousarray(idx, dtype=np.uint32)
    npts = np.zeros(4096, np.int32)
    xy = np.zeros((1 << 18, 2), np.int32)
    n = lib().abh_contours(idx.ctypes.data_as(_u32p), len(idx), W, H, npts.ctypes.data_as(_ip),
                           xy.ctypes.data_as(_ip), len(npts), len(xy))
    if n < 0:
        raise RuntimeError("contour probe capacity exceeded")
    out, o = [], 0
    for k in range(n):
        out.append(xy[o:o + npts[k]].copy())
        o += npts[k]
    return out


def binarize_threshold(hist, P, tozero):
    hist = np.ascontiguousarray(hist, dtype=np.uint32)
    return int(lib().abh_binarize_threshold(hist.ctypes.data_as(_u32p), int(P), int(tozero)))


def entropy(hist, nbins, P):
    hist = np.ascontiguousarray(hist, dtype=np.uint32)
    return float(lib().abh_entropy(hist.ctypes.data_as(_u32p), nbins, int(P)))


def blob_stats(xy):
    xy = np.ascontiguousarray(xy, dtype=np.int32)
    out = (C.c_double * 8)()
    lib().abh_blob_stats(xy.ctypes.data_as(_ip), len(xy), out)
    return dict(zip(("x", "y", "w", "h", "area", "m00", "m10", "m01"), list(out)))


def best_match(num, wsum2, tmpl):
    L = lib()
    num = np.ascontiguousarray(num, dtype=np.uint64)
    wsum2 = np.ascontiguousarray(wsum2, dtype=np.uint64)
    tmpl = np.ascontiguousarray(tmpl, dtype=np.uint8)
    rh, rw = num.shape
    bx, by = C.c_float(), C.c_float()
    L.abh_best_match(num.ctypes.data_as(_u64p), wsum2.ctypes.data_as(_u64p), rw, rh, tmpl.ctypes.data_as(_u8p),
                     tmpl.shape[1], tmpl.shape[0], C.byref(bx), C.byref(by))
    return bx.value, by.value


class Significance:
    def __init__(self, tss):
        self._h = lib().abh_sig_new()
        self.tss = tss
        self.loc_thres = C.c_int(3)

    def __call__(self, hist, P, store):
        hist = np.ascontiguousarray(hist, dtype=np.uint32)
        return float(lib().abh_sig_eval(self._h, hist.ctypes.data_as(_u32p), int(P), 1 if store else 0, self.tss,
                                        C.byref(self.loc_thres)))

    def __del__(self):
        try:
            lib().abh_sig_free(self._h)
        except Exception:
            pass


class Pipeline:

    def __init__(self, device, W, H, F, E, ncams, tss, nthreads=16, maskdir=""):
        L = lib()
        t = (C.c_int * len(tss))(*tss)
        self.S = E * ncams
        self._h = L.abh_pipe_new(device, W, H, F, E, ncams, t, nthreads, maskdir.encode())
        if not self._h:
            raise RuntimeError("abh_pipe_new failed (see stderr)")

    def close(self):
        if self._h:
            lib().abh_pipe_free(self._h)
            self._h = None

    def __del__(self):
        try:
            self.close()
        except Exception:
            pass

    def set_sigma(self, sigma):
        lib().abh_pipe_set_sigma(self._h, sigma.data_ptr() if hasattr(sigma, "data_ptr") else int(sigma))

    def run(self, frames, mu, sigma6, stream=0, sigma=None):
        p = [x.data_ptr() if hasattr(x, "data_ptr") else int(x) for x in (frames, mu, sigma6)]
        if sigma is not None:
            self.set_sigma(sigma)
        rc = lib().abh_pipe_run(self._h, p[0], p[1], p[2], stream)
        if rc != 0:
            raise RuntimeError("pipeline: " + lib().abh_pipe_error().decode())

    def run_host(self, frames_host, mu, sigma6):
        L = lib()
        p =[x.data_ptr() if hasattr(x, "data_ptr") else int(x) for x in (frames_host, mu, sigma6)]
        if L.abh_pipe_run_host(self._h, p[0], p[1], p[2]) != 0:
            raise RuntimeError("pipeline: " + L.abh_pipe_error().decode())

    def timing(self):
        out = (C.c_double * 12)()
        rounds = lib().abh_pipe_timing(self._h, out)
        return dict(zip(("stage1_ms", "stage2_ms", "stage3_ms", "stage4_ms", "total_ms", "s3_gpu_ms", "s3_list_ms",
                         "s3_bucket_ms", "pairs", "trigger_jobs", "dropin_stacks", "jobs_completed_on_demand"), list(out)),
                    rounds=rounds)

    def set_option(self, name, value):
        L = lib()
        if L.abh_pipe_set_option(self._h, name.encode(), int(value)) != 0:
            raise ValueError(L.abh_pipe_error().decode())

    def blob_stats(self):
        out = (C.c_double * 8)()
        lib().abh_pipe_blob_stats(self._h, out)
        v = list(out)
        keys = ("candidates", "foreground", "kept", "components", "kept_components", "large_slots")
        d = {k: int(x) for k, x in zip(keys, v)}
        d.update(otsu_ms=v[6], k4b_ms=v[7])
        return d

    def bellows_stats(self):
        out = (C.c_double * 5)()
        lib().abh_pipe_bellows(self._h, out)
        v = list(out)
        return {"vetoed": int(v[0]), "match_jobs": int(v[1]), "match_launches": int(v[2]), "residual_images": int(v[3]),
                "veto_ms": v[4]}

    def result(self, s):
        return _read_result(lib().abh_pipe_stack(self._h, s), with_dz=False)

    def summary(self):
        L = lib()
        o = (C.c_int * 6)()
        out = []
        for s in range(self.S):
            L.abh_result_state(L.abh_pipe_stack(self._h, s), o)
            out.append((o[0], o[1], o[5]))
        return out


class PipelineRing:

    def __init__(self, n, device, W, H, F, E, ncams, tss, nthreads=16, maskdir=""):
        self.device = device
        self.pipes = [Pipeline(device, W, H, F, E, ncams, tss, nthreads=nthreads, maskdir=maskdir) for _ in range(max(1, n))]

    def close(self):
        for p in self.pipes:
            p.close()

    def run_batches(self, batches, mu, sigma6, stream=0, on_done=None, host=False):
        import threading

        n = len(self.pipes)
        tms, errs = [], []
        lock = threading.Lock()

        def drive(i):
            try:
                try:
                    import torch

                    torch.cuda.set_device(self.device)
                except ImportError:
                    pass
                for k in range(i, len(batches), n):
                    if host:
                        self.pipes[i].run_host(batches[k], mu, sigma6)
                    else:
                        self.pipes[i].run(batches[k], mu, sigma6, stream)
                    if on_done:
                        on_done(k, self.pipes[i])
                    with lock:
                        tms.append(self.pipes[i].timing())
            except BaseException as e:
                errs.append(e)

        if n == 1:
            drive(0)
        else:
            th = [threading.Thread(target=drive, args=(i,)) for i in range(n)]
            for t in th:
                t.start()
            for t in th:
                t.join()
        if errs:
            raise errs[0]
        return tms
```

autobub3hs_amd/host/pipeline.cpp:

```cpp
#include <algorithm>
#include <atomic>
#include <condition_variable>
#include <deque>
#include <functional>
#include <mutex>
#include <cstdio>
#include <cstdlib>
#include <cstring>
#include <exception>
#include <memory>
#include <stdexcept>
#include <string>
#include <thread>
#include <vector>

#include <hip/hip_runtime_api.h>

#include "AlgorithmTraining/Trainer.hpp"
#include "AnalyzerUnit.hpp"
#include "BubbleLocalizer/L3Localizer.hpp"
#include "ParseFolder/Parser.hpp"
#include "common/CommonParameters.h"
#include "PICOFormatWriter/PICOFormatWriterV4.hpp"
#include "devctx.hpp"
// ... 250 lines not shown
        {
            std::lock_guard<std::mutex> lock(mu);
            batches.push_back(batch);
        }
        cv.notify_all();
        runBatch(*batch);
        std::unique_lock<std::mutex> lock(mu);
        batch->done.wait(lock, [&] { return batch->remaining == 0; });
        for (auto it = batches.begin(); it != batches.end(); ++it)
            if (it->get() == batch.get()) {
                batches.erase(it);
                break;
            }
    }

private:
    struct Batch {
        int n = 0;
        const std::function<void(int)> *fn = nullptr;
        std::atomic<int> next{0};
        int remaining = 0;
        std::condition_variable done;
    };
    void runBatch(Batch &b)
    {
        int finished = 0;
        for (;;) {
            const int i = b.next.fetch_add(1);
            if (i >= b.n)
                break;
            (*b.fn)(i);
            ++finished;
        }
        if (finished) {
            std::lock_guard<std::mutex> lock(mu);
            b.remaining -= finished;
            if (b.remaining == 0)
                b.done.notify_all();
        }
    }
    void workerLoop()
    {
        std::unique_lock<std::mutex> lock(mu);
        for (;;) {
            std::shared_ptr<Batch> pick;
            for (auto &b : batches)
                if (b->next.load() < b->n) {
                    pick = b;
                    break;
                }
            if (pick) {
                lock.unlock();
                runBatch(*pick);
                lock.lock();
                continue;
            }
            if (stop)
                return;
            cv.wait(lock);
        }
    }
    std::mutex mu;
    std::condition_variable cv;
    std::deque<std::shared_ptr<Batch>> batches;
    std::vector<std::thread> workers;
    bool stop = false;
};

}

struct CandidateList {
    uint32_t cap = 0;
    DeviceArray<uint32_t> pairs;
    DeviceArray<uint32_t> gscratch;
    Mirror<uint32_t> count, goff, gidx;
    Mirror<uint8_t> gval;
    int keptImages = 0, keptW = 0, keptH = 0;
    Mirror<uint32_t> kidx;
    DeviceArray<uint8_t> keptScratch;
    size_t keptScratchBytes = 0;

    void allocate(size_t nimg)
    {
        count.allocate(1);
        gscratch.allocate(2 * nimg);
        goff.allocate(nimg + 1);
    }
    void grow(uint32_t c)
    {
        cap = 0;
        pairs.allocate(2 * (size_t)c);
        gidx.allocate(c);
        gval.allocate(c);
        if (keptImages)
            growKept(c);
        cap = c;
    }
    void keep(int nimg, int W, int H)
    {
        keptImages = nimg;
        keptW = W;
        keptH = H;
        growKept(cap);
    }
    void growKept(uint32_t c)
    {
        keptScratchBytes = abub_label_blobs_scratch_bytes(keptImages, keptW, keptH, c, 0);
        if (keptScratchBytes == 0)
            throw std::runtime_error("RunPipeline: frame size not supported by the blob labelling");
        keptScratch.allocate(keptScratchBytes);
        kidx.allocate(c);
    }
    void group(int nimg, const uint32_t *d_hist, const int32_t *d_thr, hipStream_t s, const char *what)
    {
        check(abub_pairs_group_hist_dev(pairs, count.d, cap, nimg, gscratch, goff.d, gidx.d, gval.d, d_hist, d_thr, s), what);
    }
    void offsetsToHost(int nimg, hipStream_t s)
    {
        count.toHost(1, s);
        goff.toHost((size_t)nimg + 1, s);
    }
    bool fits(int attempt, const char *what)
    {
        const uint32_t n = *count.h;
        if (n <= cap)
            return true;
        if (attempt > 0 || n > (1u << 30))
            throw std::runtime_error(std::string("RunPipeline: ") + what);
        grow(n + n / 4 + 1024);
        return false;
    }
    void pairsToHost(hipStream_t s)
    {
        if (const uint32_t n = *count.h) {
            gidx.toHost(n, s);
            gval.toHost(n, s);
        }
    }
    void bind(PlannedImage &p, int k) const
    {
        p.fg = gidx.h + goff.h[k];
        p.fgv = gval.h + goff.h[k];
        p.nfg = goff.h[k + 1] - goff.h[k];
    }
};

struct PipeStats {
    double stage1Ms = 0, stage2Ms = 0, stage3Ms = 0, stage4Ms = 0, s3GpuMs = 0, s3ListMs = 0;
    int rounds = 0;
    uint32_t pairs = 0;
    double totalMs = 0;
    long long jobsLaunched = 0;
    long long jobsCompleted = 0;
    int dropIns = 0;
    int vetoed = 0, matchJobs = 0, matchLaunches = 0, residualImages = 0;
    double vetoMs = 0;
    long long blobCandidates = 0, blobForeground = 0, blobKept = 0, blobComponents = 0, blobKeptComponents = 0, blobLargeSlots = 0;
    double blobOtsuMs = 0, blobK4bMs = 0;

    void reset() { *this = PipeStats(); }
    void merge(const PipeStats &g)
    {
        stage1Ms = std::max(stage1Ms, g.stage1Ms);
        stage2Ms = std::max(stage2Ms, g.stage2Ms);
        stage3Ms = std::max(stage3Ms, g.stage3Ms);
        stage4Ms = std::max(stage4Ms, g.stage4Ms);
        s3GpuMs = std::max(s3GpuMs, g.s3GpuMs);
        s3ListMs = std::max(s3ListMs, g.s3ListMs);
        rounds = std::max(rounds, g.rounds);
        pairs += g.pairs;
        vetoed += g.vetoed;
        matchJobs += g.matchJobs;
        matchLaunches += g.matchLaunches;
        residualImages += g.residualImages;
        vetoMs += g.vetoMs;
        blobCandidates += g.blobCandidates;
        blobForeground += g.blobForeground;
        blobKept += g.blobKept;
        blobComponents += g.blobComponents;
        blobKeptComponents += g.blobKeptComponents;
        blobLargeSlots += g.blobLargeSlots;
        blobOtsuMs += g.blobOtsuMs;
        blobK4bMs += g.blobK4bMs;
    }
};

struct Group {
    int s0 = 0, s1 = 0;
    Event stage1Done, kernelsDone, blockDone;
    struct Fetch {
        int first = 0, n = 0;
        size_t pieceOff = 0;
        bool deferred = false;
    };
    struct Block {
        Mirror<abub_job> jobs;
        Mirror<uint32_t> hist;
        DeviceArray<uint64_t> pieces;
        DeviceArray<uint32_t> pcount;
        Mirror<uint8_t> inc, want;
        size_t pieceCap = 0, pieceUsed = 0;
        int slots = 0;
        int used = 0;
        std::vector<Fetch> fetches;
    };
    std::vector<Block> blocks;
    Mirror<abub_job> jobs3;
    Mirror<uint32_t> hist3;
    DeviceArray<uint8_t> img;
    Mirror<int32_t> thr;
    CandidateList list;
    struct Blobs {
        bool ready = false;
        Mirror<int32_t> otsu, minbox;
        Mirror<uint32_t> koff, kstats;
        DeviceArray<uint32_t> ncomp, nkc, coff;
        Event ev[3];
    } blobs;
    struct Veto {
        int capJobs = 0;
        size_t scratchBytes = 0;
        Mirror<uint32_t> fidx;
        Mirror<float> xy;
        DeviceArray<uint8_t> scratch;
        int capImg = 0;
        Mirror<uint8_t> rend;
        DeviceArray<uint8_t> syn, img;
        DeviceArray<uint32_t> rhist;
        Mirror<uint32_t> hist;
        Mirror<abub_job> jobs;
        Mirror<int32_t> thr;
        CandidateList list;
        std::vector<std::pair<cv::Mat, DeviceArray<uint8_t>>> templates;
    } veto;
    int nthreads = 1;
    PipeStats stats;
    std::string error;
    Stream stream;
};

class RunPipeline {
public:
    int device, W, H, F, E, C, S, nthreads, ngroups;
    size_t P;
    std::vector<int> tss;
    std::string maskDir;
    DeviceArray<uint8_t> ownFrames;
    std::vector<Group> groups;
    std::unique_ptr<WorkerPool> pool;
    std::vector<int> blocks;
    bool deferPieces = false;
    bool bellowsDropIn = false;
    PipeStats stats;
    Stream stage1Stream;
    int chainStride = 0;
    bool ordered = true;
    int pairCap = 0;
    int blobs = 0;
    std::mutex launchMu;
    std::vector<StackState> stacks;
    std::vector<std::unique_ptr<Trainer>> trainers;
    MemParser parser;
    std::vector<StackMeta> meta;
    MemParser metaParser;
    const uint8_t *d_sigmaRaw = nullptr;
    Stream copyStream;
    std::vector<Event> copied;
    bool waitCopies = false;

    void setStackMeta(std::vector<StackMeta> &&m)
    {
        if ((int)m.size() != S)
            throw std::runtime_error("RunPipeline::setStackMeta: one entry per stack expected");
        meta = std::move(m);
        metaParser = MemParser();
        for (int s = 0; s < S; ++s) {
            if ((int)meta[s].names.size() > F || meta[s].ok.size() != meta[s].names.size())
                throw std::runtime_error("RunPipeline::setStackMeta: stack longer than the pipeline's frame count");
            metaParser.AddNamedFrames(meta[s].eventID, s % C, meta[s].names);
        }
    }
    void writeEvent(int k, int eventNumber, OutputWriter &out)
    {
        StagedBubbles staged;
        for (int c = 0; c < C; ++c) {
            const StackState &ss = stacks[(size_t)k * C + c];
            if (!ss.error.empty())
                std::cout << ss.error << '\n';
            staged.stage(out, ss, c, eventNumber);
        }
        out.writeCameraOutput();
    }
    abub_job triggerJob(int s, int i, uint32_t out) const
    {
        const int c = s % C, off = refOffset(tss[c]);
        const int Fs = meta.empty() ? F : (int)meta[s].names.size();
        const int last = std::max(Fs - 1, 0);
        abub_job j;
        j.cur = (uint32_t)(s * F + std::min(i, last));
        j.ref = (uint32_t)(s * F + std::min(std::max(i - off, 0), last));
        j.model = (uint32_t)c;
        j.out = out;
        return j;
    }
    void bindBlock(Group::Block &B, int k, StackState &st_, int f, int q)
    {
        const Group::Fetch &fe = B.fetches[f];
        const size_t blen = (size_t)(blocks[k + 1] - blocks[k]), slot = (size_t)fe.first + q;
        st_.data.bh[k] = B.hist.h + slot * blen * 256;
        st_.data.inc[k] = fe.deferred ? B.inc.h + slot * blen : nullptr;
        st_.data.fetchOf[k] = f;
        st_.data.slotOf[k] = q;
    }
    int launchBlock(Group::Block &B, int k, const std::vector<int> &list, const uint8_t *d_frames, const uint8_t *d_sigma6,
                    hipStream_t stream)
    {
        const int a = blocks[k], blen = blocks[k + 1] - blocks[k];
        const int first = B.used, n = (int)list.size();
        if (blen <= 0 || n == 0)
            return first;
        if (first + n > B.slots)
            throw std::runtime_error("RunPipeline: a frame block was requested twice for one stack");
        const size_t j0 = (size_t)first * blen;
        for (int q = 0; q < n; ++q)
            for (int i = 0; i < blen; ++i)
                B.jobs.h[j0 + (size_t)q * blen + i] = triggerJob(list[q], a + i, (uint32_t)((size_t)q * blen + i));
        abub_job *dj = B.jobs.d + j0;
        uint32_t *dh = B.hist.d + j0 * 256;
        const int nj = n * blen;
        B.jobs.toDevice(nj, stream, j0);
        Group::Fetch fe;
        fe.first = first;
        fe.n = n;
        const bool defer = deferPieces && abub_k2_deferred_ok(W, H);
        const size_t pcap = defer ? abub_k2_pieces_cap(nj, W, H) : 0;
        if (defer && B.fetches.size() < 64 && B.pieceUsed + pcap <= B.pieceCap) {
            fe.deferred = true;
            fe.pieceOff = B.pieceUsed;
            B.pieceUsed += pcap;
            check(abub_diff_hist_chained_deferred_dev(d_frames, d_sigma6, dj, nj, W, H, dh, blen, chainStride,
                                                      B.pieces + fe.pieceOff, (uint32_t)pcap, B.pcount + B.fetches.size(),
                                                      B.inc.d + j0, stream),
                  "trigger search K2 (deferred pieces)");
            B.inc.toHost(nj, stream, j0);
        } else {
            check(chainStride > 0 ? abub_diff_hist_chained_dev(d_frames, d_sigma6, dj, nj, W, H, dh, blen, chainStride, stream)
                                  : abub_diff_hist_dev(d_frames, d_sigma6, dj, nj, W, H, dh, nullptr, 0, stream),
                  "trigger search K2");
        }
        B.hist.toHost((size_t)nj * 256, stream, j0 * 256);
        B.fetches.push_back(fe);
        B.used = first + n;
        stats.jobsLaunched += nj;
        return first;
    }

    RunPipeline(int device_, int W_, int H_, int F_, int E_, int C_, const int *tss_, int nthreads_, const char *maskdir)
        : device(device_), W(W_), H(H_), F(F_), E(E_), C(C_), S(E_ * C_), nthreads(nthreads_), P((size_t)W_ * H_),
          tss(tss_, tss_ + C_), maskDir(maskdir ? maskdir : "")
    {
        if (W <= 0 || H <= 0 || F <= 0 || E <= 0 || C <= 0)
            throw std::runtime_error("RunPipeline: bad geometry");
        HIPOK(hipSetDevice(device));
        const char *eg = getenv("ABUB_PIPE_GROUPS");
        ngroups = eg ? atoi(eg) : 1;
        const char *ebw = getenv("ABUB_PIPE_BELLOWS");
        bellowsDropIn = ebw && std::string(ebw) == "dropin";
        const char *eo = getenv("ABUB_PIPE_ORDERED");
        ordered = eo ? atoi(eo) != 0 : true;
        const char *eb = getenv("ABUB_PIPE_BLOBS");
        blobs = eb ? atoi(eb) != 0 : 0;
        int prLow = 0, prHigh = 0;
        HIPOK(hipDeviceGetStreamPriorityRange(&prLow, &prHigh));
        stage1Stream.create(prLow);
        if (ngroups < 1)
            ngroups = 1;
        if (ngroups > S)
            ngroups = S;
        const int K = NumFramesBubbleTrack + 1;
        chainStride = chainStrideOf(tss.data(), C);
        groups.resize(ngroups);
        pool.reset(new WorkerPool(std::max(0, nthreads - ngroups)));
        {
            const char *el = getenv("ABUB_PIPE_LAZY");
            const bool lazy = el ? atoi(el) != 0 : true;
            const char *e0 = getenv("ABUB_PIPE_BLOCK0"), *e1 = getenv("ABUB_PIPE_BLOCK");
            int first = e0 && atoi(e0) > 0 ? atoi(e0) : F / 2 + 4, step = e1 && atoi(e1) > 0 ? atoi(e1) : std::max(4, F / 5);
            blocks.clear();
            blocks.push_back(1);
            if (lazy && F > 8)
                for (int b = std::min(first + 1, F); b < F && (int)blocks.size() < BatchEventData::MAXB; b += step)
                    blocks.push_back(b);
            blocks.push_back(std::max(F, 1));
            const char *ed = getenv("ABUB_PIPE_DEFER");
            deferPieces = (ed ? atoi(ed) != 0 : true) && chainStride > 0 && abub_fast_path(W) != 0;
        }
        const int nB = (int)blocks.size() - 1;
        const char *ec = getenv("ABUB_PIPE_PAIRCAP");
        pairCap = ec ? atoi(ec) : 0;
        for (int g = 0; g < ngroups; ++g) {
            Group &G = groups[g];
            G.s0 = (int)((long long)S * g / ngroups);
            G.s1 = (int)((long long)S * (g + 1) / ngroups);
            const size_t ns = (size_t)(G.s1 - G.s0), n3 = ns * K;
            G.nthreads = std::max(1, nthreads / ngroups);
            G.stream.create(prHigh);
            G.stage1Done.create(false);
            G.kernelsDone.create(false);
            G.blockDone.create(false);
            G.blocks.resize(nB);
            for (int k = 0; k < nB; ++k) {
                Group::Block &B = G.blocks[k];
                const size_t nj = ns * (size_t)std::max(blocks[k + 1] - blocks[k], 1);
                B.slots = (int)ns;
                B.jobs.allocate(nj);
                B.hist.allocate(nj * 256);
                B.pieceCap = deferPieces ? nj * (size_t)(H / 16 + 8) : 1;
                B.pieces.allocate(B.pieceCap);
                B.pcount.allocate(64);
                B.inc.allocate(nj);
                B.want.allocate(nj);
            }
            G.jobs3.allocate(n3);
            G.hist3.allocate(n3 * 256);
            G.img.allocate(abub_fast_path(W) ? 256 : n3 * P);
            G.thr.allocate(n3);
            G.list.allocate(n3);
            G.list.grow(pairCap > 0 ? (uint32_t)pairCap : (8u << 20) / ngroups);
        }
        for (int c = 0; c < C; ++c) {
            trainers.emplace_back(new Trainer(c, {}, "", "cam%d_image%u.png", "", parser.clone(), false));
            trainers.back()->TrainingSetSize = tss[c];
            trainers.back()->ModelId = 0;
        }
        std::vector<cv::Mat> none((size_t)F);
        for (int e = 0; e < E; ++e)
            for (int c = 0; c < C; ++c)
                parser.AddFrames(std::to_string(e), c, none, 10000);
    }

    ~RunPipeline()
    {
        (void)hipSetDevice(device);
        for (Group &G : groups)
            (void)abub_scratch_release(G.stream.get());
        (void)abub_scratch_release(stage1Stream.get());
    }

    void runFromHost(const uint8_t *h_frames, const uint8_t *d_mu, const uint8_t *d_sigma6)
    {
        HIPOK(hipSetDevice(device));
        if (!ownFrames) {
            ownFrames.allocate((size_t)S * F * P);
            copied.resize(ngroups);
            for (Event &e : copied)
                e.create(false);
        }
        for (int g = 0; g < ngroups; ++g) {
            const Group &G = groups[g];
            const size_t off = (size_t)G.s0 * F * P, n = (size_t)(G.s1 - G.s0) * F * P;
            HIPOK(hipMemcpyAsync(ownFrames + off, h_frames + off, n, hipMemcpyHostToDevice, copyStream.get()));
            HIPOK(hipEventRecord(copied[g].get(), copyStream.get()));
        }
        waitCopies = true;
        run(ownFrames, d_mu, d_sigma6, nullptr);
        waitCopies = false;
    }

    void run(const uint8_t *d_frames, const uint8_t *d_mu, const uint8_t *d_sigma6, hipStream_t callerStream)
    {
        HIPOK(hipSetDevice(device));
        if (!waitCopies)
            HIPOK(hipStreamSynchronize(callerStream));
        g_quietAnalyzers = true;
        double t0 = nowMs();
        stacks.clear();
        stacks.resize(S);
        stats.reset();
        for (size_t gi = 0; gi < groups.size(); ++gi) {
            Group &G = groups[gi];
            if (waitCopies)
                HIPOK(hipStreamWaitEvent(stage1Stream.get(), copied[gi].get(), 0));
            for (Group::Block &B : G.blocks) {
                B.used = 0;
                B.pieceUsed = 0;
                B.fetches.clear();
            }
            std::vector<int> all;
            for (int sI = G.s0; sI < G.s1; ++sI)
                all.push_back(sI);
            if (F > 1)
                launchBlock(G.blocks[0], 0, all, d_frames, d_sigma6, stage1Stream.get());
            HIPOK(hipEventRecord(G.stage1Done.get(), stage1Stream.get()));
        }
        std::vector<std::thread> th;
        for (int g = 1; g < ngroups; ++g)
            th.emplace_back([&, g]() { runGroupNoThrow(groups[g], d_frames, d_mu, d_sigma6); });
        runGroupNoThrow(groups[0], d_frames, d_mu, d_sigma6);
        for (auto &t : th)
            t.join();
        for (int s = 0; s < S; ++s)
            if (stacks[s].dropIn) {
                ++stats.dropIns;
                runDropIn(s, d_frames, d_mu);
            }
        for (Group &G : groups) {
            if (!G.error.empty())
                throw std::runtime_error(G.error);
            stats.merge(G.stats);
        }
        stats.totalMs = nowMs() - t0;
    }

private:
    void runDropIn(int s, const uint8_t *d_frames, const uint8_t *d_mu)
    {
        StackState &st_ = stacks[s];
        st_.bubbles.clear();
        if (!d_sigmaRaw) {
            st_.staged = -6;
            st_.error = "bellows veto needs the drop-in path, but no sigma image was given to the pipeline";
            return;
        }
        const int e = s / C, c = s % C;
        try {
            const int Fs = meta.empty() ? F : (int)meta[s].names.size();
            std::vector<cv::Mat> frames((size_t)Fs);
            for (int i = 0; i < Fs; ++i) {
                if (!meta.empty() && !meta[s].ok[i])
                    continue;
                frames[i].create(H, W, CV_8U);
                HIPOK(hipMemcpy(frames[i].data, d_frames + ((size_t)s * F + i) * P, P, hipMemcpyDeviceToHost));
            }
            MemParser mp;
            const std::string evName = meta.empty() ? std::to_string(e) : meta[s].eventID;
            if (meta.empty())
                mp.AddFrames(evName, c, frames, 10000);
            else
                mp.AddNamedFrames(evName, c, meta[s].names, &frames);
            Trainer t(c, {}, "", "cam%d_image%u.png", "", mp.clone(), false);
            t.TrainedAvgImage.create(H, W, CV_8U);
            t.TrainedSigmaImage.create(H, W, CV_8U);
            HIPOK(hipMemcpy(t.TrainedAvgImage.data, d_mu + (size_t)c * P, P, hipMemcpyDeviceToHost));
            HIPOK(hipMemcpy(t.TrainedSigmaImage.data, d_sigmaRaw + (size_t)c * P, P, hipMemcpyDeviceToHost));
            t.TrainingSetSize = tss[c];
            t.ModelId = 0;
            Trainer *tp = &t;
            L3Localizer A(evName, "", c, true, &tp, maskDir, mp.clone());
            st_.staged = analyzeUntilBubble(&A, true, "", st_.error);
            if (st_.staged != -6)
                st_.capture(A);
        } catch (std::exception &ex) {
            st_.error = ex.what();
            st_.staged = -6;
        }
        DeviceContext::releaseThread();
    }

    void runGroupNoThrow(Group &G, const uint8_t *d_frames, const uint8_t *d_mu, const uint8_t *d_sigma6)
    {
        G.error.clear();
        try {
            (void)hipSetDevice(device);
            runGroup(G, d_frames, d_mu, d_sigma6);
        } catch (std::exception &e) {
            G.error = e.what();
        }
    }

    void runGroup(Group &G, const uint8_t *d_frames, const uint8_t *d_mu, const uint8_t *d_sigma6)
    {
        G.stats.reset();
        const int ns = G.s1 - G.s0;
        double t0 = nowMs();
        pool->parallelFor(ns, [&](int k) {
            const int s = G.s0 + k;
            StackState &st_ = stacks[s];
            const int e = s / C, c = s % C;
            Trainer *t = trainers[c].get();
            if (meta.empty()) {
                st_.analyzer.reset(new L3Localizer(std::to_string(e), "", c, true, &t, maskDir, parser.clone()));
                st_.data.F = F;
                st_.data.ok = nullptr;
            } else {
                st_.analyzer.reset(new L3Localizer(meta[s].eventID, "", c, true, &t, maskDir, metaParser.clone()));
                st_.data.F = (int)meta[s].names.size();
                st_.data.ok = meta[s].ok.data();
            }
            st_.data.W = W;
            st_.data.H = H;
            st_.data.refOffset = refOffset(tss[c]);
            st_.data.bellowsDropIn = bellowsDropIn;
            st_.data.clearVeto();
            st_.vetoed = false;
            st_.data.nblocks = (int)blocks.size() - 1;
            for (size_t b = 0; b < blocks.size(); ++b)
                st_.data.bstart[b] = blocks[b];
            for (int b = 0; b < st_.data.nblocks; ++b) {
                st_.data.bh[b] = nullptr;
                st_.data.inc[b] = nullptr;
            }
            if (F > 1)
                bindBlock(G.blocks[0], 0, st_, 0, k);
            st_.analyzer->AttachEventData(&st_.data);
        });
        HIPOK(hipEventSynchronize(G.stage1Done.get()));
        G.stats.stage1Ms = nowMs() - t0;

        std::vector<int> pending(ns);
        for (int k = 0; k < ns; ++k)
            pending[k] = G.s0 + k;
        while (!pending.empty()) {
            ++G.stats.rounds;
            double t2 = nowMs();
            std::vector<int> todo(pending);
            while (!todo.empty()) {
                pool->parallelFor((int)todo.size(), [&](int k) { triggerAndPlan(stacks[todo[k]]); });
                std::vector<int> need;
                for (int sI : todo)
                    if (stacks[sI].needMore)
                        need.push_back(sI);
                if (need.empty())
                    break;
                fetchBlocks(G, need, d_frames, d_sigma6);
                todo.swap(need);
            }
            G.stats.stage2Ms += nowMs() - t2;
            double t3 = nowMs();
            std::vector<int> loc;
            for (int s : pending)
                if (stacks[s].localize)
                    loc.push_back(s);
            if (!loc.empty())
                batchImages(G, loc, d_frames, d_mu, d_sigma6);
            G.stats.stage3Ms += nowMs() - t3;
            double t4 = nowMs();
            pool->parallelFor((int)loc.size(), [&](int k) { localize(stacks[loc[k]]); });
            vetoRound(G, loc, d_frames, d_sigma6);
            G.stats.stage4Ms += nowMs() - t4;
            std::vector<int> next;
            for (int s : pending)
                if (!stacks[s].done)
                    next.push_back(s);
            pending.swap(next);
        }
        pool->parallelFor(ns, [&](int k) {
            StackState &st_ = stacks[G.s0 + k];
            st_.capture(*st_.analyzer);
            st_.analyzer.reset();
        });
    }

    void fetchBlocks(Group &G, const std::vector<int> &need, const uint8_t *d_frames, const uint8_t *d_sigma6)
    {
        hipStream_t stream = ordered ? stage1Stream.get() : G.stream.get();
        const int nB = (int)blocks.size() - 1;
        std::vector<std::vector<int>> byBlock((size_t)nB);
        std::vector<std::vector<std::vector<int>>> byFetch((size_t)nB);
        for (int sI : need) {
            const BatchEventData &d = stacks[sI].data;
            if (!d.needPieces)
                byBlock[(size_t)d.needBlock].push_back(sI);
            else {
                auto &v = byFetch[(size_t)d.needBlock];
                if (v.size() <= (size_t)d.fetchOf[d.needBlock])
                    v.resize((size_t)d.fetchOf[d.needBlock] + 1);
                v[(size_t)d.fetchOf[d.needBlock]].push_back(sI);
            }
        }
        std::vector<int> newFetch((size_t)nB, -1);
        {
            std::lock_guard<std::mutex> lock(launchMu);
            for (int k = 0; k < nB; ++k) {
                Group::Block &B = G.blocks[k];
                if (!byBlock[k].empty()) {
                    launchBlock(B, k, byBlock[k], d_frames, d_sigma6, stream);
                    newFetch[k] = (int)B.fetches.size() - 1;
                }
                const size_t blen = (size_t)(blocks[k + 1] - blocks[k]);
                for (size_t f = 0; f < byFetch[k].size(); ++f) {
                    if (byFetch[k][f].empty())
                        continue;
                    const Group::Fetch &fe = B.fetches[f];
                    const size_t nj = (size_t)fe.n * blen, base = (size_t)fe.first * blen;
                    uint8_t *hw = B.want.h + base;
                    std::memset(hw, 0, nj);
                    for (int sI : byFetch[k][f]) {
                        BatchEventData &d = stacks[sI].data;
                        for (size_t j = (size_t)(d.needFrame - blocks[k]); j < blen; ++j)
                            if (d.inc[k][j]) {
                                hw[(size_t)d.slotOf[k] * blen + j] = 1;
                                ++stats.jobsCompleted;
                            }
                    }
                    B.want.toDevice(nj, stream, base);
                    check(abub_diff_hist_pieces_dev(d_frames, d_sigma6, B.jobs.d + base, (int)nj, W, H, B.hist.d + base * 256,
                                                    B.pieces + fe.pieceOff, B.pcount + f, B.want.d + base, stream),
                          "trigger search K2 (pieces)");
                    for (int sI : byFetch[k][f]) {
                        BatchEventData &d = stacks[sI].data;
                        const size_t j0 = (size_t)(d.needFrame - blocks[k]), o = (base + (size_t)d.slotOf[k] * blen + j0) * 256;
                        B.hist.toHost((blen - j0) * 256, stream, o);
                    }
                }
            }
            HIPOK(hipEventRecord(G.blockDone.get(), stream));
        }
        HIPOK(hipEventSynchronize(G.blockDone.get()));
        for (int k = 0; k < nB; ++k) {
            for (size_t q = 0; q < byBlock[k].size(); ++q) {
                StackState &st_ = stacks[byBlock[k][q]];
                bindBlock(G.blocks[k], k, st_, newFetch[k], (int)q);
                st_.needMore = false;
            }
            const size_t blen = (size_t)(blocks[k + 1] - blocks[k]);
            for (auto &v : byFetch[k])
                for (int sI : v) {
                    StackState &st_ = stacks[sI];
                    for (size_t j = (size_t)(st_.data.needFrame - blocks[k]); j < blen; ++j)
                        st_.data.inc[k][j] = 0;
                    st_.needMore = false;
                }
        }
    }

    void triggerAndPlan(StackState &st_)
    {
        st_.localize = false;
        st_.needMore = false;
        AnalyzerUnit *A = st_.analyzer.get();
        try {
            size_t pixSize[256];
            const bool havePix = A->pix_counts.size() == 256;
            for (int b = 0; havePix && b < 256; ++b)
                pixSize[b] = A->pix_counts[b].size();
            const int trig0 = A->MatTrigFrame, loc0 = A->loc_thres, status0 = A->TriggerFrameIdentificationStatus;
            const bool ok0 = A->okToProceed;
            try {
                A->FindTriggerFrame(true, A->MatTrigFrame + 1);
            } catch (NeedMoreFrames &) {
                for (int b = 0; havePix && b < 256 && A->pix_counts.size() == 256; ++b)
                    A->pix_counts[b].resize(pixSize[b]);
                A->MatTrigFrame = trig0;
                A->loc_thres = loc0;
                A->TriggerFrameIdentificationStatus = status0;
                A->okToProceed = ok0;
                st_.needMore = true;
                return;
            }
            if (!A->okToProceed) {
                st_.staged = A->TriggerFrameIdentificationStatus;
                st_.done = true;
                return;
            }
            const int F = st_.data.F;
            if (F <= 5) {
                A->LocalizeOMatic("");
                st_.staged = -8;
                st_.done = true;
                return;
            }
            const int t = A->MatTrigFrame;
            const int off = refOffset(A->TrainedData->TrainingSetSize);
            st_.data.planned.clear();
            st_.data.cur = nullptr;
            st_.data.clearVeto();
            PlannedImage g;
            g.kind = 0;
            g.i = t;
            g.ref = std::max(t - off, 0);
            g.tozero = A->loc_thres;
            g.slot = -1;
            g.thr = 0;
            g.minBox = -1;
            st_.data.planned.push_back(g);
            const int last = (t < 29) ? NumFramesBubbleTrack : (39 - t);
            for (int k = 1; k <= last; ++k) {
                if (t + k >= F)
                    break;
                PlannedImage p;
                p.kind = 1;
                p.i = t + k;
                p.ref = 0;
                p.tozero = 3;
                p.slot = -1;
                p.thr = 0;
                p.minBox = kTrackMinBoxArea;
                st_.data.planned.push_back(p);
            }
            st_.localize = true;
        } catch (std::exception &e) {
            st_.error = e.what();
            st_.staged = -6;
            st_.done = true;
        }
    }

    void batchImages(Group &G, const std::vector<int> &loc, const uint8_t *d_frames, const uint8_t *d_mu,
                     const uint8_t *d_sigma6)
    {
        hipStream_t stream = ordered ? stage1Stream.get() : G.stream.get();
        hipStream_t back = G.stream.get();
        int nd = 0, np = 0;
        for (int s : loc)
            for (PlannedImage &p : stacks[s].data.planned)
                (p.kind == 0 ? nd : np)++;
        std::vector<int> order(loc);
        std::stable_sort(order.begin(), order.end(), [&](int a, int b) { return a % C < b % C; });
        int di = 0, pi = nd;
        for (int s : order) {
            const int c = s % C;
            for (PlannedImage &p : stacks[s].data.planned) {
                p.slot = p.kind == 0 ? di++ : pi++;
                abub_job &j = G.jobs3.h[p.slot];
                j.cur = (uint32_t)(s * F + p.i);
                j.ref = (uint32_t)(s * F + p.ref);
                j.model = (uint32_t)c;
                j.out = (uint32_t)(p.kind == 0 ? p.slot : p.slot - nd);
            }
        }
        const int nimg = nd + np;
        double ta = nowMs();
        const bool useBlobs = blobs != 0;
        Group::Blobs &B = G.blobs;
        CandidateList &L = G.list;
        if (useBlobs)
            initBlobs(G);
        std::vector<PlannedImage *> bySlot((size_t)nimg);
        for (int s : loc) {
            stacks[s].data.roundHists = G.hist3.h;
            for (PlannedImage &p : stacks[s].data.planned) {
                bySlot[p.slot] = &p;
                G.thr.h[p.slot] = p.tozero;
                if (useBlobs)
                    B.minbox.h[p.slot] = p.minBox;
            }
        }
        for (int attempt = 0;; ++attempt) {
            G.jobs3.toDevice(nimg, stream);
            G.thr.toDevice(nimg, stream);
            HIPOK(hipMemsetAsync(L.count.d, 0, sizeof(uint32_t), stream));
// ... 287 lines not shown
        HIPOK(hipStreamSynchronize(st));
        for (int k = 0; k < n; ++k) {
            const int s = req[k].first;
            BatchEventData::ResidualMemo &r = *req[k].second;
            std::memcpy(r.hist, V.hist.h + (size_t)k * 256, sizeof(r.hist));
            PlannedImage &p = r.img;
            p.kind = 2;
            p.i = r.trig;
            p.ref = r.pre;
            p.slot = k;
            p.tozero = V.thr.h[k];
            p.thr = binarizeThresholdFromHist(r.hist, P, p.tozero);
            p.minBox = -1;
            L.bind(p, k);
            r.ready = true;
            if (!stacks[s].vetoed) {
                stacks[s].vetoed = true;
                ++G.stats.vetoed;
            }
        }
        G.stats.residualImages += n;
        return true;
    }

    void initBlobs(Group &G)
    {
        Group::Blobs &B = G.blobs;
        if (B.ready)
            return;
        const size_t n3 = (size_t)(G.s1 - G.s0) * (NumFramesBubbleTrack + 1);
        B.otsu.allocate(n3);
        B.minbox.allocate(n3);
        B.koff.allocate(n3 + 1);
        B.ncomp.allocate(n3);
        B.nkc.allocate(n3);
        B.coff.allocate(n3 + 1);
        B.kstats.allocate(4);
        for (Event &e : B.ev)
            e.create(true);
        G.list.keep((int)n3, W, H);
        B.ready = true;
    }

    void localize(StackState &st_)
    {
        st_.needBellows = false;
        AnalyzerUnit *A = st_.analyzer.get();
        try {
            A->LocalizeOMatic("");
            if (!A->okToProceed) {
                st_.staged = -8;
                st_.done = true;
                return;
            }
            st_.staged = A->BubbleList.empty() ? -1 : 0;
            st_.done = !A->BubbleList.empty();
        } catch (NeedBellows &) {
            st_.needBellows = true;
        } catch (NeedsDropInPath &) {
            st_.dropIn = true;
            st_.done = true;
        } catch (std::exception &e) {
            st_.error = e.what();
            st_.staged = -6;
            st_.done = true;
        }
    }
};

void RunPipelineDelete::operator()(RunPipeline *p) const { delete p; }

RunPipelinePtr newRunPipeline(int device, int W, int H, int F, int E, int C, const int *tss, int nthreads, const char *maskDir)
{
    return RunPipelinePtr(new RunPipeline(device, W, H, F, E, C, tss, nthreads, maskDir));
}
void setSigmaRaw(RunPipeline &p, const uint8_t *d_sigma) { p.d_sigmaRaw = d_sigma; }
bool setTrainingSetSizes(RunPipeline &p, const int *tss)
{
    if (chainStrideOf(tss, p.C) != p.chainStride)
        return false;
    for (int c = 0; c < p.C; ++c) {
        p.tss[c] = tss[c];
        p.trainers[c]->TrainingSetSize = tss[c];
    }
    return true;
}
void setStackMeta(RunPipeline &p, std::vector<StackMeta> &&meta) { p.setStackMeta(std::move(meta)); }
void run(RunPipeline &p, const uint8_t *d_frames, const uint8_t *d_mu, const uint8_t *d_sigma6, hipStream_t stream)
{
    p.run(d_frames, d_mu, d_sigma6, stream);
}
void writeEvent(RunPipeline &p, int k, int eventNumber, OutputWriter &out) { p.writeEvent(k, eventNumber, out); }
int bellowsVetoed(const RunPipeline &p) { return p.stats.vetoed; }

}

extern "C" {

void *abh_pipe_new(int device, int W, int H, int F, int E, int C, const int *tss, int nthreads, const char *maskdir)
{
    try {
        return new abub::RunPipeline(device, W, H, F, E, C, tss, nthreads, maskdir);
    } catch (std::exception &e) {
        fprintf(stderr, "abh_pipe_new: %s\n", e.what());
        return nullptr;
    }
}

void abh_pipe_free(void *p) { delete (abub::RunPipeline *)p; }

static thread_local std::string g_pipeErr;
const char *abh_pipe_error() { return g_pipeErr.c_str(); }

void abh_pipe_set_sigma(void *p, const void *sigma_dev) { ((abub::RunPipeline *)p)->d_sigmaRaw = (const uint8_t *)sigma_dev; }

int abh_pipe_run(void *p, const void *frames_dev, const void *mu_dev, const void *sigma6_dev, void *stream)
{
    try {
        ((abub::RunPipeline *)p)->run((const uint8_t *)frames_dev, (const uint8_t *)mu_dev, (const uint8_t *)sigma6_dev,
                                      (hipStream_t)stream);
        return 0;
    } catch (std::exception &e) {
        g_pipeErr = e.what();
        return -1;
    }
}

int abh_pipe_run_host(void *p, const void *frames_host, const void *mu_dev, const void *sigma6_dev)
{
    try {
        ((abub::RunPipeline *)p)->runFromHost((const uint8_t *)frames_host, (const uint8_t *)mu_dev, (const uint8_t *)sigma6_dev);
        return 0;
    } catch (std::exception &e) {
        g_pipeErr = e.what();
        return -1;
    }
}

const void *abh_pipe_stack(void *p, int s)
{
    const abub::StackResult &res = ((abub::RunPipeline *)p)->stacks[s];
    return &res;
}

void abh_pipe_bellows(void *p, double *out)
{
    const abub::PipeStats &st = ((abub::RunPipeline *)p)->stats;
    const double v[5] = {(double)st.vetoed, (double)st.matchJobs, (double)st.matchLaunches, (double)st.residualImages, st.vetoMs};
    std::memcpy(out, v, sizeof v);
}

int abh_pipe_set_option(void *p, const char *name, int value)
{
    if (!name || std::string(name) != "blobs") {
        g_pipeErr = std::string("abh_pipe_set_option: unknown option ") + (name ? name : "(null)");
        return -1;
    }
    if (value != 0 && value != 1) {
        g_pipeErr = "abh_pipe_set_option: blobs takes 0 or 1";
        return -1;
    }
    if (!p) {
        g_pipeErr = "abh_pipe_set_option: no pipeline";
        return -1;
    }
    ((abub::RunPipeline *)p)->blobs = value;
    return 0;
}

void abh_pipe_blob_stats(void *p, double *out)
{
    const abub::PipeStats &st = ((abub::RunPipeline *)p)->stats;
    const double v[8] = {(double)st.blobCandidates, (double)st.blobForeground, (double)st.blobKept, (double)st.blobComponents,
                         (double)st.blobKeptComponents, (double)st.blobLargeSlots, st.blobOtsuMs, st.blobK4bMs};
    std::memcpy(out, v, sizeof v);
}

int abh_pipe_timing(void *p, double *out)
{
    const abub::PipeStats &st = ((abub::RunPipeline *)p)->stats;
    const double v[12] = {st.stage1Ms, st.stage2Ms, st.stage3Ms, st.stage4Ms, st.totalMs, st.s3GpuMs, st.s3ListMs,
                          0.0,
                          (double)st.pairs, (double)st.jobsLaunched, (double)st.dropIns, (double)st.jobsCompleted};
    std::memcpy(out, v, sizeof v);
    return st.rounds;
}
}
```

include/abub_hip.h:

```cpp
#ifndef ABUB_HIP_H
#define ABUB_HIP_H

#include <stddef.h>
#include <stdint.h>

#ifdef __cplusplus
extern "C" {
#endif

#define ABUB_OK 0
#define ABUB_E_INVALID (-1)
#define ABUB_E_HIP (-2)
#define ABUB_E_NODEVICE (-3)
#define ABUB_E_OVERFLOW (-4)

typedef struct {
    uint32_t cur;
    uint32_t ref;
    uint32_t model;
    uint32_t out;
} abub_job;

const char *abub_last_error(void);
int abub_device_count(void);
int abub_device_info(int device, char *name, int name_cap, int *cus, uint64_t *hbm_bytes);


int abub_sigma6_dev(const uint8_t *sigma, uint8_t *sigma6, size_t n, void *stream);

int abub_fill_stack_jobs_dev(abub_job *jobs, int nstacks, int F, int first, int count, int ref_offset,
                             int nmodels, void *stream);

int abub_diff_hist_dev(const uint8_t *frames, const uint8_t *sigma6, const abub_job *jobs, int njobs,
                       int W, int H, uint32_t *hist, uint8_t *diff, int rows_per_chunk, void *stream);

int abub_diff_roi_dev(const uint8_t *cur, const uint8_t *ref, const uint8_t *sigma6, int W, int H,
                      int rx, int ry, int rw, int rh, uint8_t *diff, uint32_t *hist, void *stream);

int abub_train_dev(const uint8_t *frames, const uint32_t *idx, int N, int W, int H, uint8_t *mu,
                   uint8_t *sigma, void *stream);

int abub_pair_hist_dev(const uint8_t *frames, const abub_job *pairs, int npairs, int W, int H,
                       uint32_t *hist, void *stream);

int abub_posttrig_dev(const uint8_t *frames, const uint8_t *mu, const uint8_t *sigma6,
                      const abub_job *jobs, int njobs, int W, int H, uint32_t *hist, uint8_t *img,
                      void *stream);

int abub_fg_compact_dev(const uint8_t *img, int nimg, int W, int H, const int32_t *thr,
                        uint32_t *idx, int cap, uint32_t *count, void *stream);

int abub_fast_path(int W);

int abub_diff_hist_chained_dev(const uint8_t *frames, const uint8_t *sigma6, const abub_job *jobs, int njobs, int W,
                               int H, uint32_t *hist, int chain_len, int chain_stride, void *stream);

int abub_diff_hist_chained_store_dev(const uint8_t *frames, const uint8_t *sigma6, const abub_job *jobs, int njobs, int W,
                                     int H, uint32_t *hist, uint8_t *diff, int chain_len, int chain_stride, void *stream);

size_t abub_k2_pieces_cap(int njobs, int W, int H);
int abub_diff_hist_chained_deferred_dev(const uint8_t *frames, const uint8_t *sigma6, const abub_job *jobs, int njobs, int W,
                                        int H, uint32_t *hist, int chain_len, int chain_stride, void *pieces,
                                        uint32_t pieces_cap, uint32_t *npieces, uint8_t *incomplete, void *stream);
int abub_diff_hist_pieces_dev(const uint8_t *frames, const uint8_t *sigma6, const abub_job *jobs, int njobs, int W, int H,
                              uint32_t *hist, const void *pieces, const uint32_t *npieces, const uint8_t *want, void *stream);

int abub_k2_set_option(const char *name, int value);

int abub_k2_deferred_ok(int W, int H);

int abub_k3_set_option(const char *name, int value);

int abub_scratch_release(void *stream);

int abub_bound_counts_dev(void *stream, uint32_t counts[2]);
int abub_diff_hist_compact_dev(const uint8_t *frames, const uint8_t *sigma6, const abub_job *jobs, int njobs,
                               int W, int H, uint32_t *hist, uint8_t *diff, const int32_t *cthr,
                               uint32_t *pairs, uint32_t cap, uint32_t *count, uint32_t slot_base,
                               void *stream);
int abub_posttrig_compact_dev(const uint8_t *frames, const uint8_t *mu, const uint8_t *sigma6,
                              const abub_job *jobs, int njobs, int W, int H, uint32_t *hist, uint8_t *img,
                              const int32_t *cthr, uint32_t *pairs, uint32_t cap, uint32_t *count,
                              uint32_t slot_base, void *stream);

int abub_pairs_group_dev(const uint32_t *pairs, const uint32_t *count, uint32_t cap, int nslots,
                         uint32_t *scratch , uint32_t *offsets ,
                         uint32_t *idx_out , uint8_t *val_out , void *stream);

int abub_pairs_group_hist_dev(const uint32_t *pairs, const uint32_t *count, uint32_t cap, int nslots,
                              uint32_t *scratch, uint32_t *offsets, uint32_t *idx_out, uint8_t *val_out,
                              const uint32_t *hist , const int32_t *cthr ,
                              void *stream);

int abub_fg_compact_pairs_dev(const uint8_t *img, int nimg, int W, int H, const int32_t *thr,
                              uint32_t *pairs, uint32_t cap, uint32_t *count, void *stream);

int abub_binarize_thr_dev(const uint32_t *hist, const int32_t *tozero, int nslots, int W, int H, int32_t *thr, void *stream);

typedef struct abub_blob {
    uint32_t first;
    int32_t x0, y0, x1, y1;
    uint32_t npix;
} abub_blob;

int abub_label_blobs_dev(const uint32_t *offsets, const uint32_t *idx, const uint8_t *val, uint32_t in_cap, int nslots, int W,
                         int H, const int32_t *thr, const int32_t *min_box_area, uint32_t *kept_off, uint32_t *kept_idx,
                         uint32_t cap, uint32_t *ncomp, uint32_t *nkept_comp, uint32_t *comp_off, abub_blob *comp,
                         uint32_t comp_cap, uint32_t *stats, void *scratch, size_t scratch_bytes, void *stream);
size_t abub_label_blobs_scratch_bytes(int nslots, int W, int H, uint32_t in_cap, int with_comp);

int abub_match_ccorr_dev(const uint8_t *img, int W, int H, const uint8_t *tmpl, int tw, int th,
                         unsigned long long *num, unsigned long long *wsum2, void *stream);
int abub_match_ccorr_batch_dev(const uint8_t *frames, int W, int H, const uint32_t *frame_idx, int njobs,
                               const uint8_t *tmpl, int tw, int th, unsigned long long *num, unsigned long long *wsum2,
                               void *stream);
int abub_match_best_batch_dev(const uint8_t *frames, int W, int H, const uint32_t *frame_idx, int njobs,
                              const uint8_t *tmpl, int tw, int th, float *best_xy, void *scratch, size_t scratch_bytes,
                              void *stream);
size_t abub_match_best_scratch_bytes(int W, int H, int tw, int th, int njobs);
int abub_subsat_hist_dev(uint8_t *img, const uint8_t *sub, int W, int H, uint32_t *hist, void *stream);


typedef struct abub_ctx abub_ctx;

int abub_ctx_create(abub_ctx **out, int device, int W, int H, int max_frames);
void abub_ctx_destroy(abub_ctx *ctx);

int abub_ctx_train(abub_ctx *ctx, const uint8_t *const *frames, int N, uint8_t *mu_out,
                   uint8_t *sigma_out);
int abub_ctx_pair_hist(abub_ctx *ctx, const uint8_t *f0, const uint8_t *f1, uint32_t hist[256]);

int abub_ctx_set_model(abub_ctx *ctx, const uint8_t *mu, const uint8_t *sigma);

int abub_ctx_upload_stack(abub_ctx *ctx, const uint8_t *const *frames, int F);

int abub_ctx_diff_hist_batch(abub_ctx *ctx, int ref_offset, int first, int count, uint32_t *hist_out);

int abub_ctx_diff_frame(abub_ctx *ctx, int i, int ref, uint8_t *D_out, uint32_t *hist_out);

int abub_ctx_diff_frame_roi(abub_ctx *ctx, int i, int ref, int rx, int ry, int rw, int rh, uint8_t *D_out,
                            uint32_t *hist_out);

int abub_ctx_posttrig(abub_ctx *ctx, int i, uint8_t *O_out, uint32_t *hist_out);

int abub_ctx_foreground(abub_ctx *ctx, int thr, uint32_t *idx_out, int cap, int *n);

int abub_ctx_match_template(abub_ctx *ctx, int i, const uint8_t *tmpl, int tw, int th, unsigned long long *num_out,
                            unsigned long long *wsum2_out);
int abub_ctx_subtract_image(abub_ctx *ctx, const uint8_t *sub, uint32_t *hist_out);
int abub_ctx_set_image(abub_ctx *ctx, const uint8_t *img);

int abub_ctx_fetch_image(abub_ctx *ctx, uint8_t *out);

typedef struct abub_png_seg {
    uint32_t off;
    uint32_t len;
} abub_png_seg;
typedef struct abub_png_frame {
    uint32_t seg_begin;
    uint32_t seg_count;
    uint32_t zoff;
    uint32_t zlen;
    uint32_t lut;
    uint32_t reserved;
    uint64_t dst;
} abub_png_frame;
#define ABUB_PNG_E_DESC 1
#define ABUB_PNG_E_HEADER 2
#define ABUB_PNG_E_TRUNCATED 3
#define ABUB_PNG_E_BLOCKTYPE 4
#define ABUB_PNG_E_STORED 5
#define ABUB_PNG_E_SYMBOLS 6
#define ABUB_PNG_E_CODES 7
#define ABUB_PNG_E_NOEOB 8
#define ABUB_PNG_E_CODE 9
#define ABUB_PNG_E_DISTANCE 10
#define ABUB_PNG_E_TOOMUCH 11
#define ABUB_PNG_E_TOOLITTLE 12
#define ABUB_PNG_E_ADLER 13
#define ABUB_PNG_E_FILTER 14
#define ABUB_PNG_E_INTERNAL 15
size_t abub_png_raw_stride(int W, int H);
int abub_png_decode_dev(const uint8_t *files, size_t files_bytes, const abub_png_frame *frames, int nframes,
                        const abub_png_seg *segs, int nsegs, const uint8_t *luts, int nluts, int W, int H,
                        uint8_t *zbuf, size_t zbuf_bytes, uint8_t *rawbuf, size_t rawbuf_bytes, uint8_t *out,
                        size_t out_bytes, int32_t *status, void *stream);

#ifdef __cplusplus
}
#endif
#endif
```

Baseline: 3.517 million.

## Gate trigger-pass diff jobs past a device-detected trigger frame per stack

Adds a device kernel that sums the nonzero histogram counts per frame, spots the first sustained jump over a quiet baseline, and writes a per-stack gate frame. Later chained diff/histogram launches hand over any job whose current frame lies beyond that gate instead of computing it. The host tracks stacks where the real trigger turns out to need frames past the gate and completes those on demand. This cuts trigger-pass work on frames after the trigger, at the cost of an extra small kernel, a heuristic threshold that may miss, and more branching in the kernels.

```diff
diff --git a/autobub3hs_amd/_lib.py b/autobub3hs_amd/_lib.py
--- a/autobub3hs_amd/_lib.py
+++ b/autobub3hs_amd/_lib.py
@@ -45,6 +45,8 @@
     "abub_png_raw_stride": (_sz, [_i, _i]),
     "abub_png_decode_dev": (_i, [_vp, _sz, _vp, _i, _vp, _i, _vp, _i, _i, _i, _vp, _sz, _vp, _sz, _vp, _sz, _vp, _vp]),
     "abub_diff_hist_chained_deferred_dev": (_i, [_vp, _vp, _vp, _i, _i, _i, _vp, _i, _i, _vp, C.c_uint32, _vp, _vp, _vp]),
+    "abub_diff_hist_chained_gated_dev": (_i, [_vp, _vp, _vp, _i, _i, _i, _vp, _i, _i, _vp, C.c_uint32, _vp, _vp, _vp, _i, _vp]),
+    "abub_trigger_gate_dev": (_i, [_vp, _vp, _i, _i, _i, _i, _i, _i, _i, _vp, _vp, _vp, _vp, _i, _vp]),
     "abub_diff_hist_pieces_dev": (_i, [_vp, _vp, _vp, _i, _i, _i, _vp, _vp, _vp, _vp, _vp]),
     "abub_diff_hist_compact_dev": (_i, [_vp, _vp, _vp, _i, _i, _i, _vp, _vp, _vp, _vp, C.c_uint32, _vp, C.c_uint32, _vp]),
     "abub_posttrig_compact_dev": (_i, [_vp, _vp, _vp, _vp, _i, _i, _i, _vp, _vp, _vp, _vp, C.c_uint32, _vp, C.c_uint32, _vp]),
diff --git a/autobub3hs_amd/csrc/abub_dev.hpp b/autobub3hs_amd/csrc/abub_dev.hpp
--- a/autobub3hs_amd/csrc/abub_dev.hpp
+++ b/autobub3hs_amd/csrc/abub_dev.hpp
@@ -468,4 +468,6 @@
     uint32_t df_cap = 0;
     uint32_t *df_count = nullptr;
     uint8_t *df_incomplete = nullptr;
+    const int32_t *gate = nullptr;
+    int gateF = 0;
 };
diff --git a/autobub3hs_amd/csrc/abub_k2.hip b/autobub3hs_amd/csrc/abub_k2.hip
--- a/autobub3hs_amd/csrc/abub_k2.hip
+++ b/autobub3hs_amd/csrc/abub_k2.hip
@@ -498,7 +498,8 @@
                                                     uint32_t *__restrict__ hist, uint8_t *__restrict__ diff,
                                                     const int32_t *__restrict__ cthr, uint32_t *pairs, uint32_t pcap,
                                                     uint32_t *pcount, uint32_t slot_base, SusList gl,
-                                                    uint8_t *__restrict__ incomplete)
+                                                    uint8_t *__restrict__ incomplete,
+                                                    const int32_t *__restrict__ gate, int gateF, int gateL)
 {
     constexpr int NP = 2 * NDW;
     __shared__ uint32_t pend[K2B_PEND];
@@ -507,6 +508,14 @@
     const int job = unit / nchunks;
     const int chunk = unit - job * nchunks;
     const abub_job jb = jobs[job];
+    if (gate) {
+        const int g = gate[job / gateL];
+        if (g >= 0 && (int)(jb.cur % (uint32_t)gateF) > g) {
+            const int gy0 = chunk * rows_per_chunk, gy1 = gy0 + rows_per_chunk < H ? gy0 + rows_per_chunk : H;
+            k2b_hand_over(units, nunits, (uint32_t)unit, gy0, gy1, lane, incomplete, (uint32_t)job);
+            return;
+        }
+    }
     const size_t P = (size_t)W * H;
     const uint8_t *cur = frames + (size_t)jb.cur * P;
     const uint8_t *ref = frames + (size_t)jb.ref * P;
@@ -586,7 +595,8 @@
                                                    int H, int rows_per_chunk, int nchunks, uint32_t budget,
                                                    uint2 *__restrict__ units, uint32_t *__restrict__ nunits,
                                                    uint32_t *__restrict__ hist, uint8_t *__restrict__ diff, SusList gl,
-                                                   int syncD, uint8_t *__restrict__ incomplete)
+                                                   int syncD, uint8_t *__restrict__ incomplete,
+                                                   const int32_t *__restrict__ gate, int gateF)
 {
     using Job = K2BoundJob<NDW, false, true>;
     extern __shared__ uint32_t k2c_lds[];
@@ -618,7 +628,7 @@
         K2C_PUBLISH(0x7fffffff);
         return;
     }
-    const int k = nr - slot * K < K ? nr - slot * K : K;
+    int k = nr - slot * K < K ? nr - slot * K : K;
     Job J[K];
     abub_job jb[K];
     const uint32_t jidx0 = (uint32_t)(blk * L + r + S * slot * K);
@@ -629,6 +639,30 @@
     int y1 = y0 + rows_per_chunk;
     if (y1 > H)
         y1 = H;
+    if (gate) {
+        const int g = gate[blk];
+        if (g >= 0) {
+            int ka = k;
+#pragma unroll
+            for (int t = K - 1; t >= 0; t--)
+                if (t < k && (int)(jb[t].cur % (uint32_t)gateF) > g)
+                    ka = t;
+#pragma unroll
+            for (int t = 0; t < K; t++)
+                if (t >= ka && t < k)
+                    k2b_hand_over(units, nunits, (jidx0 + (uint32_t)(S * t)) * (uint32_t)nchunks + (uint32_t)chunk, y0, y1, lane,
+                                  incomplete, jidx0 + (uint32_t)(S * t));
+            if (ka == 0) {
+                K2C_PUBLISH(0x7fffffff);
+                return;
+            }
+#pragma unroll
+            for (int t = 1; t < K; t++)
+                if (t >= ka)
+                    jb[t] = jb[t - 1];
+            k = ka;
+        }
+    }
     bool chained = true;
 #pragma unroll
     for (int t = 1; t < K; t++)
@@ -1004,7 +1038,7 @@
             constexpr bool CAN_SPLIT = NDW >= 5 && NDW <= 7;
             const bool split = CAN_SPLIT && opt.split;
             const bool pf2 = NDW == 5 && split && Kc == 4 && (opt.scanpf < 0 || opt.scanpf == 2);
-#define K2C_ARGS frames, sigma6, jobs, L, S, nwgs, W, H, R, nchunks, budget, units, npieces, hist, diff, gl, syncD, ca.df_incomplete
+#define K2C_ARGS frames, sigma6, jobs, L, S, nwgs, W, H, R, nchunks, budget, units, npieces, hist, diff, gl, syncD, ca.df_incomplete, ca.gate, ca.gateF
 #define K2C_LAUNCH_SP(KK, SP, PFD) \
     hipLaunchKernelGGL((k2_sad_chain<NDW, KK, SP, PFD>), grid, dim3(64 * NW), ldsBytes, st, K2C_ARGS)
 #define K2C_LAUNCH(KK)                                                                                              \
@@ -1028,7 +1062,7 @@
 #define K2S_LAUNCH(CO)                                                                                              \
     hipLaunchKernelGGL((k2_bound_scan<NDW, CO>), dim3((unsigned)nunits), dim3(64), 0, st, frames, sigma6, jobs, W, H, \
                        R, nchunks, budget, units, npieces, hist, diff, ca.cthr, ca.pairs, ca.cap, ca.count,         \
-                       ca.slot_base, gl, ca.df_incomplete)
+                       ca.slot_base, gl, ca.df_incomplete, ca.gate, ca.gateF, L > 0 ? L : 1)
             if (ca.cthr) {
                 K2S_LAUNCH(true);
             } else {
@@ -1206,6 +1240,26 @@
     return diff_hist_impl(frames, sigma6, jobs, njobs, W, H, hist, nullptr, 0, ca, stream);
 }
 
+extern "C" int abub_diff_hist_chained_gated_dev(const uint8_t *frames, const uint8_t *sigma6, const abub_job *jobs, int njobs,
+                                                int W, int H, uint32_t *hist, int chain_len, int chain_stride, void *pieces,
+                                                uint32_t pieces_cap, uint32_t *npieces, uint8_t *incomplete,
+                                                const int32_t *gate, int F, void *stream)
+{
+    if (chain_len < 0 || chain_stride < 0 || !pieces || !npieces || !incomplete || !pick_ndw(W) || !k2_options().bound || !gate ||
+        F <= 0 || (chain_len > 0 && njobs % chain_len != 0))
+        return set_err(ABUB_E_INVALID, "abub_diff_hist_chained_gated_dev: bad arguments (or no bound-and-verify pass for this width)");
+    CompactArgs ca = {nullptr, nullptr, 0, nullptr, 0};
+    ca.chain_len = chain_len;
+    ca.chain_stride = chain_stride;
+    ca.df_pieces = (uint2 *)pieces;
+    ca.df_cap = pieces_cap;
+    ca.df_count = npieces;
+    ca.df_incomplete = incomplete;
+    ca.gate = gate;
+    ca.gateF = F;
+    return diff_hist_impl(frames, sigma6, jobs, njobs, W, H, hist, nullptr, 0, ca, stream);
+}
+
 template <int NDW>
 static void launch_pieces(const uint8_t *frames, const uint8_t *sigma6, const abub_job *jobs, int W, int H, int R, int nchunks,
                           uint32_t *hist, const uint2 *pieces, const uint32_t *npieces, const uint8_t *want, unsigned grid,
diff --git a/autobub3hs_amd/csrc/abub_misc.hip b/autobub3hs_amd/csrc/abub_misc.hip
--- a/autobub3hs_amd/csrc/abub_misc.hip
+++ b/autobub3hs_amd/csrc/abub_misc.hip
@@ -88,6 +88,69 @@
         return ABUB_OK;
     hipLaunchKernelGGL(k_fill_stack_jobs, dim3((n + 255) / 256), dim3(256), 0, (hipStream_t)stream,
                        jobs, nstacks, F, first, count, ref_offset, nmodels);
+    HIPCHK(hipGetLastError());
+    return ABUB_OK;
+}
+
+#define ABUB_GATE_LEAD 4
+#define ABUB_GATE_SLACK 3
+__global__ __launch_bounds__(64) void k_trigger_gate(const uint32_t *__restrict__ hist, const uint8_t *__restrict__ incomplete,
+                                                     int count, int first, int njobs, int frame0, uint32_t quiet,
+                                                     uint32_t *__restrict__ nz, uint8_t *__restrict__ flagged,
+                                                     const int32_t *__restrict__ gate_in, int32_t *__restrict__ gate_out, int force)
+{
+    const int s = blockIdx.x, l = threadIdx.x;
+    uint32_t *mynz = nz + (size_t)s * njobs;
+    uint8_t *myfl = flagged + (size_t)s * njobs;
+    for (int q = 0; q < count; q++) {
+        const uint32_t *h = hist + ((size_t)s * count + q) * 256;
+        uint32_t v = h[l + 64] + h[l + 128] + h[l + 192] + (l ? h[l] : 0u);
+        for (int o = 32; o > 0; o >>= 1)
+            v += __shfl_xor(v, o);
+        if (l == 0) {
+            mynz[first + q] = v;
+            myfl[first + q] = incomplete ? incomplete[(size_t)s * count + q] : 0;
+        }
+    }
+    if (l != 0)
+        return;
+    int g = gate_in ? gate_in[s] : -1;
+    if (force >= 0)
+        g = force;
+    const int known = first + count;
+    if (g < 0 && known > ABUB_GATE_LEAD) {
+        bool ok = true;
+        for (int j = 0; j < ABUB_GATE_LEAD; j++)
+            ok = ok && !myfl[j] && mynz[j] <= quiet;
+        uint32_t sum = 0, n = 0;
+        for (int j = 0; ok && j + 1 < known; j++) {
+            if (n >= ABUB_GATE_LEAD) {
+                const uint32_t mean = sum / n, bound = mean + (mean >> 1) + 16u;
+                if (mynz[j] > bound && mynz[j + 1] > bound) {
+                    g = frame0 + j + ABUB_GATE_SLACK;
+                    break;
+                }
+            }
+            if (myfl[j])
+                break;
+            sum += mynz[j];
+            n++;
+        }
+    }
+    gate_out[s] = g;
+}
+
+extern "C" int abub_trigger_gate_dev(const uint32_t *hist, const uint8_t *incomplete, int nstacks, int count, int first,
+                                     int njobs, int frame0, int W, int H, uint32_t *nz, uint8_t *flagged, const int32_t *gate_in,
+                                     int32_t *gate_out, int force, void *stream)
+{
+    if (!hist || !nz || !flagged || !gate_out || nstacks < 0 || count <= 0 || first < 0 || first + count > njobs || W <= 0 || H <= 0)
+        return set_err(ABUB_E_INVALID, "abub_trigger_gate_dev: bad arguments");
+    if (nstacks == 0)
+        return ABUB_OK;
+    const uint32_t quiet = (uint32_t)(((size_t)W * H) >> 12) + 32u;
+    hipLaunchKernelGGL(k_trigger_gate, dim3(nstacks), dim3(64), 0, (hipStream_t)stream, hist, incomplete, count, first, njobs,
+                       frame0, quiet, nz, flagged, gate_in, gate_out, force);
     HIPCHK(hipGetLastError());
     return ABUB_OK;
 }
diff --git a/autobub3hs_amd/hip.py b/autobub3hs_amd/hip.py
--- a/autobub3hs_amd/hip.py
+++ b/autobub3hs_amd/hip.py
@@ -74,6 +74,30 @@
                                                               _ptr(incomplete), _stream()),
                "abub_diff_hist_chained_deferred_dev")
     return hist, (pieces, npieces, incomplete)
+
+
+def diff_hist_gated(frames, sigma6_, jobs, W, H, chain, gate, F):
+    _need_cuda(frames, sigma6_, jobs, gate)
+    n = jobs.shape[0]
+    hist = torch.empty((n, 256), dtype=torch.int32, device=frames.device)
+    cap = int(_lib.lib().abub_k2_pieces_cap(n, W, H))
+    pieces = torch.empty((max(cap, 1), 2), dtype=torch.int32, device=frames.device)
+    npieces = torch.zeros((1,), dtype=torch.int32, device=frames.device)
+    incomplete = torch.empty((n,), dtype=torch.uint8, device=frames.device)
+    _lib.check(_lib.lib().abub_diff_hist_chained_gated_dev(_ptr(frames), _ptr(sigma6_), _ptr(jobs), n, W, H, _ptr(hist),
+                                                           int(chain[0]), int(chain[1]), _ptr(pieces), cap, _ptr(npieces),
+                                                           _ptr(incomplete), _ptr(gate), int(F), _stream()),
+               "abub_diff_hist_chained_gated_dev")
+    return hist, (pieces, npieces, incomplete)
+
+
+def trigger_gate(hist, incomplete, nstacks, count, first, njobs, W, H, nz, flagged, gate_in=None, force=-1, frame0=1):
+    _need_cuda(hist, incomplete, nz, flagged, gate_in)
+    gate = torch.empty((nstacks,), dtype=torch.int32, device=hist.device)
+    _lib.check(_lib.lib().abub_trigger_gate_dev(_ptr(hist), _ptr(incomplete), nstacks, count, first, njobs, frame0, W, H,
+                                                _ptr(nz), _ptr(flagged), _ptr(gate_in), _ptr(gate), int(force), _stream()),
+               "abub_trigger_gate_dev")
+    return gate
 
 
 def diff_hist_pieces(frames, sigma6_, jobs, W, H, hist, state, want):
diff --git a/autobub3hs_amd/host.py b/autobub3hs_amd/host.py
--- a/autobub3hs_amd/host.py
+++ b/autobub3hs_amd/host.py
@@ -62,6 +62,7 @@
     "abh_pipe_timing": (_i, [_vp, _dp]),
     "abh_pipe_set_option": (_i, [_vp, _s, _i]),
     "abh_pipe_blob_stats": (None, [_vp, _dp]),
+    "abh_pipe_gate_stats": (None, [_vp, _dp]),
     "abh_pipe_bellows": (None, [_vp, _dp]),
 }
 _lib = None
@@ -383,9 +384,11 @@
     def timing(self):
         out = (C.c_double * 12)()
         rounds = lib().abh_pipe_timing(self._h, out)
+        gate = (C.c_double * 3)()
+        lib().abh_pipe_gate_stats(self._h, gate)
         return dict(zip(("stage1_ms", "stage2_ms", "stage3_ms", "stage4_ms", "total_ms", "s3_gpu_ms", "s3_list_ms",
                          "s3_bucket_ms", "pairs", "trigger_jobs", "dropin_stacks", "jobs_completed_on_demand"), list(out)),
-                    rounds=rounds)
+                    rounds=rounds, gated_jobs=gate[0], gate_misses=gate[1], gated=gate[2])
 
     def set_option(self, name, value):
         L = lib()
diff --git a/autobub3hs_amd/host/pipeline.cpp b/autobub3hs_amd/host/pipeline.cpp
--- a/autobub3hs_amd/host/pipeline.cpp
+++ b/autobub3hs_amd/host/pipeline.cpp
@@ -426,6 +426,8 @@
     double totalMs = 0;
     long long jobsLaunched = 0;
     long long jobsCompleted = 0;
+    long long gatedJobs = 0;
+    int gateMisses = 0;
     int dropIns = 0;
     int vetoed = 0, matchJobs = 0, matchLaunches = 0, residualImages = 0;
     double vetoMs = 0;
@@ -443,6 +445,8 @@
         s3ListMs = std::max(s3ListMs, g.s3ListMs);
         rounds = std::max(rounds, g.rounds);
         pairs += g.pairs;
+        gatedJobs += g.gatedJobs;
+        gateMisses += g.gateMisses;
         vetoed += g.vetoed;
         matchJobs += g.matchJobs;
         matchLaunches += g.matchLaunches;
@@ -479,6 +483,11 @@
         std::vector<Fetch> fetches;
     };
     std::vector<Block> blocks;
+    Mirror<int32_t> gate;
+    DeviceArray<uint32_t> gateNz;
+    DeviceArray<uint8_t> gateFl;
+    bool gatedRun = false;
+    std::vector<uint8_t> gateMissed;
     Mirror<abub_job> jobs3;
     Mirror<uint32_t> hist3;
     DeviceArray<uint8_t> img;
@@ -524,6 +533,8 @@
     std::unique_ptr<WorkerPool> pool;
     std::vector<int> blocks;
     bool deferPieces = false;
+    bool gateMode = false;
+    int gateForce = -1;
     bool bellowsDropIn = false;
     PipeStats stats;
     Stream stage1Stream;
@@ -587,7 +598,7 @@
         st_.data.slotOf[k] = q;
     }
     int launchBlock(Group::Block &B, int k, const std::vector<int> &list, const uint8_t *d_frames, const uint8_t *d_sigma6,
-                    hipStream_t stream)
+                    hipStream_t stream, const int32_t *gate = nullptr, bool copies = true)
     {
         const int a = blocks[k], blen = blocks[k + 1] - blocks[k];
         const int first = B.used, n = (int)list.size();
@@ -608,25 +619,41 @@
         fe.n = n;
         const bool defer = deferPieces && abub_k2_deferred_ok(W, H);
         const size_t pcap = defer ? abub_k2_pieces_cap(nj, W, H) : 0;
+        if (gate && !(defer && B.fetches.size() < 64 && B.pieceUsed + pcap <= B.pieceCap))
+            throw std::runtime_error("RunPipeline: a gated launch needs deferred pieces");
         if (defer && B.fetches.size() < 64 && B.pieceUsed + pcap <= B.pieceCap) {
             fe.deferred = true;
             fe.pieceOff = B.pieceUsed;
             B.pieceUsed += pcap;
-            check(abub_diff_hist_chained_deferred_dev(d_frames, d_sigma6, dj, nj, W, H, dh, blen, chainStride,
-                                                      B.pieces + fe.pieceOff, (uint32_t)pcap, B.pcount + B.fetches.size(),
-                                                      B.inc.d + j0, stream),
+            check(gate ? abub_diff_hist_chained_gated_dev(d_frames, d_sigma6, dj, nj, W, H, dh, blen, chainStride,
+                                                          B.pieces + fe.pieceOff, (uint32_t)pcap, B.pcount + B.fetches.size(),
+                                                          B.inc.d + j0, gate, F, stream)
+                       : abub_diff_hist_chained_deferred_dev(d_frames, d_sigma6, dj, nj, W, H, dh, blen, chainStride,
+                                                             B.pieces + fe.pieceOff, (uint32_t)pcap, B.pcount + B.fetches.size(),
+                                                             B.inc.d + j0, stream),
                   "trigger search K2 (deferred pieces)");
-            B.inc.toHost(nj, stream, j0);
+            if (copies)
+                B.inc.toHost(nj, stream, j0);
         } else {
             check(chainStride > 0 ? abub_diff_hist_chained_dev(d_frames, d_sigma6, dj, nj, W, H, dh, blen, chainStride, stream)
                                   : abub_diff_hist_dev(d_frames, d_sigma6, dj, nj, W, H, dh, nullptr, 0, stream),
                   "trigger search K2");
         }
-        B.hist.toHost((size_t)nj * 256, stream, j0 * 256);
+        if (copies)
+            B.hist.toHost((size_t)nj * 256, stream, j0 * 256);
         B.fetches.push_back(fe);
         B.used = first + n;
         stats.jobsLaunched += nj;
         return first;
+    }
+
+    void copyBlock(Group::Block &B, int k, hipStream_t stream)
+    {
+        const Group::Fetch &fe = B.fetches.back();
+        const size_t blen = (size_t)(blocks[k + 1] - blocks[k]), j0 = (size_t)fe.first * blen, nj = (size_t)fe.n * blen;
+        if (fe.deferred)
+            B.inc.toHost(nj, stream, j0);
+        B.hist.toHost(nj * 256, stream, j0 * 256);
     }
 
     RunPipeline(int device_, int W_, int H_, int F_, int E_, int C_, const int *tss_, int nthreads_, const char *maskdir)
@@ -668,6 +695,18 @@
             blocks.push_back(std::max(F, 1));
             const char *ed = getenv("ABUB_PIPE_DEFER");
             deferPieces = (ed ? atoi(ed) != 0 : true) && chainStride > 0 && abub_fast_path(W) != 0;
+            const char *eg = getenv("ABUB_PIPE_GATE"), *eg0 = getenv("ABUB_PIPE_GATE0");
+            gateMode = lazy && deferPieces && !(e0 && *e0) && !(e1 && *e1) && (eg ? atoi(eg) != 0 : false) && F > 9;
+            if (const char *ef = getenv("ABUB_PIPE_GATE_FORCE"))
+                gateForce = *ef && atoi(ef) >= 0 ? atoi(ef) : -1;
+            if (gateMode) {
+                const int g0 =eg0 && atoi(eg0) >= 8 ? atoi(eg0) / 8 * 8 : 8;
+                blocks.clear();
+                blocks.push_back(1);
+                for (int b = 1 + g0; b < F && (int)blocks.size() < BatchEventData::MAXB; b += 8)
+                    blocks.push_back(b);
+                blocks.push_back(F);
+            }
         }
         const int nB = (int)blocks.size() - 1;
         const char *ec = getenv("ABUB_PIPE_PAIRCAP");
@@ -695,6 +734,13 @@
                 B.inc.allocate(nj);
                 B.want.allocate(nj);
             }
+            if (gateMode) {
+                G.gate.allocate((size_t)nB * ns);
+                G.gateNz.allocate(ns * (size_t)F);
+                G.gateFl.allocate(ns * (size_t)F);
+                for (size_t q = 0; q < ns; ++q)
+                    G.gate.h[q] = -1;
+            }
             G.jobs3.allocate(n3);
             G.hist3.allocate(n3 * 256);
             G.img.allocate(abub_fast_path(W) ? 256 : n3 * P);
@@ -763,7 +809,25 @@
             std::vector<int> all;
             for (int sI = G.s0; sI < G.s1; ++sI)
                 all.push_back(sI);
-            if (F > 1)
+            G.gatedRun = gateMode && abub_k2_deferred_ok(W, H);
+            if (G.gatedRun) {
+                hipStream_t st = stage1Stream.get();
+                const int nB = (int)blocks.size() - 1, ns = G.s1 - G.s0;
+                for (int k = 0; k < nB; ++k) {
+                    Group::Block &B = G.blocks[k];
+                    launchBlock(B, k, all, d_frames, d_sigma6, st, k > 0 ? G.gate.d + (size_t)k * ns : nullptr, false);
+                    if (k + 1 < nB)
+                        check(abub_trigger_gate_dev(B.hist.d, B.inc.d, ns, blocks[k + 1] - blocks[k], blocks[k] - 1, F - 1, 1, W, H,
+                                                    G.gateNz, G.gateFl, k > 0 ? G.gate.d + (size_t)k * ns : nullptr,
+                                                    G.gate.d + (size_t)(k + 1) * ns, gateForce, st),
+                              "trigger gate");
+                }
+                for (int k = 0; k < nB; ++k)
+                    copyBlock(G.blocks[k], k, st);
+                if (nB > 1)
+                    G.gate.toHost((size_t)(nB - 1) * ns, st, (size_t)ns);
+                G.gateMissed.assign((size_t)ns, 0);
+            } else if (F > 1)
                 launchBlock(G.blocks[0], 0, all, d_frames, d_sigma6, stage1Stream.get());
             HIPOK(hipEventRecord(G.stage1Done.get(), stage1Stream.get()));
         }
@@ -875,11 +939,20 @@
                 st_.data.inc[b] = nullptr;
             }
             if (F > 1)
-                bindBlock(G.blocks[0], 0, st_, 0, k);
+                for (int b = 0; b < (G.gatedRun ? st_.data.nblocks : 1); ++b)
+                    bindBlock(G.blocks[b], b, st_, 0, k);
             st_.analyzer->AttachEventData(&st_.data);
         });
         HIPOK(hipEventSynchronize(G.stage1Done.get()));
         G.stats.stage1Ms = nowMs() - t0;
+        if (G.gatedRun)
+            for (int b = 1; b + 1 < (int)blocks.size(); ++b)
+                for (int k = 0; k < ns; ++k) {
+                    const int g = G.gate.h[(size_t)b * ns + k];
+                    const int last = std::max((meta.empty() ? F : (int)meta[G.s0 + k].names.size()) - 1, 0);
+                    for (int i = blocks[b]; g >= 0 && i < blocks[b + 1]; ++i)
+                        G.stats.gatedJobs += std::min(i, last) > g;
+                }
 
         std::vector<int> pending(ns);
         for (int k = 0; k < ns; ++k)
@@ -961,6 +1034,13 @@
                     std::memset(hw, 0, nj);
                     for (int sI : byFetch[k][f]) {
                         BatchEventData &d = stacks[sI].data;
+                        if (G.gatedRun && k > 0 && !G.gateMissed[(size_t)(sI - G.s0)]) {
+                            const int g = G.gate.h[(size_t)k * (G.s1 - G.s0) + (sI - G.s0)];
+                            if (g >= 0 && std::min(d.needFrame, std::max(d.F - 1, 0)) > g) {
+                                G.gateMissed[(size_t)(sI - G.s0)] = 1;
+                                ++G.stats.gateMisses;
+                            }
+                        }
                         for (size_t j = (size_t)(d.needFrame - blocks[k]); j < blen; ++j)
                             if (d.inc[k][j]) {
                                 hw[(size_t)d.slotOf[k] * blen + j] = 1;
@@ -1554,19 +1634,27 @@
 
 int abh_pipe_set_option(void *p, const char *name, int value)
 {
-    if (!name || std::string(name) != "blobs") {
+    const bool isBlobs = name && std::string(name) == "blobs", isForce = name && std::string(name) == "gate_force";
+    if (!isBlobs && !isForce) {
         g_pipeErr = std::string("abh_pipe_set_option: unknown option ") + (name ? name : "(null)");
         return -1;
     }
-    if (value != 0 && value != 1) {
+    if (isBlobs && value != 0 && value != 1) {
         g_pipeErr = "abh_pipe_set_option: blobs takes 0 or 1";
+        return -1;
+    }
+    if (isForce && value < -1) {
+        g_pipeErr = "abh_pipe_set_option: gate_force takes a frame index, or -1 for the device's own rule";
         return -1;
     }
     if (!p) {
         g_pipeErr = "abh_pipe_set_option: no pipeline";
         return -1;
     }
-    ((abub::RunPipeline *)p)->blobs = value;
+    if (isBlobs)
+        ((abub::RunPipeline *)p)->blobs = value;
+    else
+        ((abub::RunPipeline *)p)->gateForce = value;
     return 0;
 }
 
@@ -1583,8 +1671,18 @@
     const abub::PipeStats &st = ((abub::RunPipeline *)p)->stats;
     const double v[12] = {st.stage1Ms, st.stage2Ms, st.stage3Ms, st.stage4Ms, st.totalMs, st.s3GpuMs, st.s3ListMs,
                           0.0,
-                          (double)st.pairs, (double)st.jobsLaunched, (double)st.dropIns, (double)st.jobsCompleted};
+                          (double)st.pairs, (double)(st.jobsLaunched - st.gatedJobs), (double)st.dropIns, (double)st.jobsCompleted};
     std::memcpy(out, v, sizeof v);
     return st.rounds;
 }
+
+void abh_pipe_gate_stats(void *p, double *out)
+{
+    const abub::RunPipeline *rp = (const abub::RunPipeline *)p;
+    bool gated = false;
+    for (const abub::Group &G : rp->groups)
+        gated = gated || G.gatedRun;
+    const double v[3] = {(double)rp->stats.gatedJobs, (double)rp->stats.gateMisses, gated ? 1.0 : 0.0};
+    std::memcpy(out, v, sizeof v);
 }
+}
diff --git a/include/abub_hip.h b/include/abub_hip.h
--- a/include/abub_hip.h
+++ b/include/abub_hip.h
@@ -64,6 +64,14 @@
                                         uint32_t pieces_cap, uint32_t *npieces, uint8_t *incomplete, void *stream);
 int abub_diff_hist_pieces_dev(const uint8_t *frames, const uint8_t *sigma6, const abub_job *jobs, int njobs, int W, int H,
                               uint32_t *hist, const void *pieces, const uint32_t *npieces, const uint8_t *want, void *stream);
+
+int abub_diff_hist_chained_gated_dev(const uint8_t *frames, const uint8_t *sigma6, const abub_job *jobs, int njobs, int W,
+                                     int H, uint32_t *hist, int chain_len, int chain_stride, void *pieces,
+                                     uint32_t pieces_cap, uint32_t *npieces, uint8_t *incomplete, const int32_t *gate, int F,
+                                     void *stream);
+int abub_trigger_gate_dev(const uint32_t *hist, const uint8_t *incomplete, int nstacks, int count, int first, int njobs,
+                          int frame0, int W, int H, uint32_t *nz, uint8_t *flagged, const int32_t *gate_in, int32_t *gate_out,
+                          int force, void *stream);
 
 int abub_k2_set_option(const char *name, int value);
 
diff --git a/profiles/r05/fit_gate_rule.py b/profiles/r05/fit_gate_rule.py
--- /dev/null
+++ b/profiles/r05/fit_gate_rule.py
@@ -0,0 +1,122 @@
+#!/usr/bin/env python3
+import argparse
+import json
+import os
+import sys
+from concurrent.futures import ThreadPoolExecutor
+
+import numpy as np
+
+sys.path.insert(0, os.path.join(os.path.dirname(os.path.abspath(__file__)), "..", ".."))
+from autobub3hs_amd import synth
+from oracle import pyoracle as orc
+
+GROUP = 8
+LEAD = 4
+QUIET_SHIFT = 12
+QUIET_ADD = 32
+BOUND_ADD = 16
+SLACK = 3
+
+
+def gate_rule(nz, flagged, W, H, known):
+    if known < LEAD + 1:
+        return -1
+    quiet = (W * H >> QUIET_SHIFT) + QUIET_ADD
+    for j in range(LEAD):
+        if flagged[j] or nz[j] > quiet:
+            return -1
+    s, n = 0, 0
+    for j in range(known - 1):
+        if n >= LEAD:
+            mean = s // n
+            bound = mean + (mean >> 1) + BOUND_ADD
+            if nz[j] > bound and nz[j + 1] > bound:
+                return (j + 1) + SLACK
+        if flagged[j]:
+            return -1
+        s += int(nz[j])
+        n += 1
+    return -1
+
+
+def replay(nz, flagged, W, H, F):
+    gate = -1
+    for last in range(GROUP, F - 1, GROUP):
+        if gate >= 0:
+            break
+        gate = gate_rule(nz, flagged, W, H, last)
+    return gate
+
+
+def one_stack(args):
+    W, H, F, ev, c, regime, mu_sg, dense = args
+    spec = synth.random_spec(W, H, F, ev, c, p_second=0.2, regime=regime)
+    fr = synth.render_event(W, H, spec, ev, c)
+    _, hists = orc.bench_trigger_pass(fr, mu_sg[1], 2, 1, F - 1, want_hists=True)
+    nz = hists[:, 1:].sum(axis=1).astype(np.int64)
+    a = orc.Analyzer(fr, mu_sg[0], mu_sg[1], 40)
+    a.find_trigger(1)
+    st = a.state()
+    a.close()
+    trig = st["trig"] if isinstance(st, dict) else st[0]
+    flagged = nz > dense
+    gate = replay(nz, flagged, W, H, F)
+    return dict(ev=ev, cam=c, t0=spec.t0, trig=int(trig), gate=int(gate), nz=[int(v) for v in nz])
+
+
+def main():
+    ap = argparse.ArgumentParser()
+    ap.add_argument("--width", type=int, default=1280)
+    ap.add_argument("--height", type=int, default=1024)
+    ap.add_argument("--frames", type=int, default=41)
+    ap.add_argument("--events", type=int, default=100)
+    ap.add_argument("--stride", type=int, default=6)
+    ap.add_argument("--threads", type=int, default=8)
+    ap.add_argument("--regimes", default="default,post_trigger_dense,noisy")
+    a = ap.parse_args()
+    orc.build()
+    W, H, F = a.width, a.height, a.frames
+    dense = W * H // 400
+    for regime in a.regimes.split(","):
+        models = []
+        for c in range(2):
+            tr = []
+            for e in range(20):
+                spec = synth.random_spec(W, H, F, e, c, p_second=0.2, regime=regime)
+                spec.F = 2
+                tr.append(synth.render_event(W, H, spec, e, c))
+            models.append(orc.welford(np.concatenate(tr)))
+        work = [(W, H, F, ev, c, regime, models[c], dense) for ev in range(0, a.events, a.stride) for c in range(2)]
+        with ThreadPoolExecutor(a.threads) as ex:
+            rows = list(ex.map(one_stack, work))
+        quiet, trg, nxt, miss, gated, saved = [], [], [], 0, 0, 0
+        for r in rows:
+            t = r["trig"]
+            nz = r["nz"]
+            if t >= 1:
+                quiet += nz[:max(t - 1, 0)]
+                trg.append(nz[t - 1])
+                if t < F - 1:
+                    nxt.append(nz[t])
+            else:
+                quiet += nz
+            if r["gate"] >= 0:
+                gated += 1
+                saved += max(0, (F - 1) - r["gate"])
+                if t >= 1 and min(t + 2, F - 1) > r["gate"]:
+                    miss += 1
+        def rng(v):
+            return "-" if not v else "%d..%d (median %d)" % (min(v), max(v), int(np.median(v)))
+        print(json.dumps({"regime": regime, "W": W, "H": H, "F": F, "stacks": len(rows), "quiet_nz": rng(quiet),
+                          "trigger_nz": rng(trg), "next_nz": rng(nxt), "gated_stacks": gated, "misses": miss,
+                          "jobs_saved_per_stack": saved / max(1, len(rows)),
+                          "trig_minus_t0": sorted(set(r["trig"] - r["t0"] for r in rows if r["t0"] is not None)),
+                          "gate_minus_trig": sorted(set(r["gate"] - r["trig"] for r in rows if r["gate"] >= 0))}))
+        for r in rows:
+            print("  ", json.dumps(r))
+        sys.stdout.flush()
+
+
+if __name__ == "__main__":
+    main()
```

Result: slower. 3.292 million (-6.4%).
